# esw0116/DynaVSR

Hardware: AMD Instinct MI355X
Metric: inner-loop frames/sec/GPU (EDVR-M x4, 5x3x180x320): forward leg = BASELINE.json configs[1]; the inner MAML step and the per-frame pipeline are `inner_step` / `per_frame_pipeline` (higher is better)
Workload: dtype f32; 1 GPU; EDVR-M x4 forward (PCD deformable alignment + TSA fusion + reconstruction), clips of 1x5x3x180x320 -> 3x720x1280 (BASELINE.json configs[1]); one step = 2 clip(s) per GPU, one per HIP stream (adapt.super_resolve_video); clips_in_flight_per_gpu=2

## Files before the change

### dynavsr_amd/_lib.py

```python
import ctypes
import os
from ctypes import POINTER, Structure, c_char_p, c_float, c_int, c_longlong, c_size_t, c_void_p

import torch

_runtime = {"configured": False, "hw_queues": None, "effective": None}


def configure_runtime(hw_queues=6):
    if not _runtime["configured"]:
        user = os.environ.get("GPU_MAX_HW_QUEUES")
        late = torch.cuda.is_initialized()
        if user is None and not late:
            os.environ["GPU_MAX_HW_QUEUES"] = str(int(hw_queues))
        _runtime.update(configured=True, hw_queues=os.environ.get("GPU_MAX_HW_QUEUES"),
                        effective=(user is not None) or not late)
    return {"hw_queues": _runtime["hw_queues"], "effective": _runtime["effective"]}


def runtime_report(device=None):
    r = configure_runtime()
    overlaps = None
    if torch.cuda.is_available():
        with torch.cuda.device(device if device is not None else torch.cuda.current_device()):
            overlaps = int(lib().dvsr_side_stream_overlaps(stream()))
    return {"hw_queues": r["hw_queues"], "effective": r["effective"], "side_stream_overlaps": overlaps}


_HERE = os.path.dirname(os.path.abspath(__file__))
SO_PATH = os.path.join(_HERE, "libdynavsr_hip.so")
_lib = None

ACT_NONE, ACT_LRELU, ACT_RELU = 0, 1, 2


class Conv2dDesc(Structure):
    _fields_ = [("x0", c_void_p), ("x1", c_void_p), ("w", c_void_p), ("bias", c_void_p),
                ("res", c_void_p), ("y", c_void_p),
                ("N", c_int), ("c0", c_int), ("c1", c_int), ("H", c_int), ("W", c_int),
                ("Cout", c_int), ("ks", c_int), ("stride", c_int), ("pad", c_int), ("act", c_int),
                ("pixel_shuffle", c_int), ("x1_bdiv", c_int),
                ("x0_bstride", c_longlong), ("x1_bstride", c_longlong),
                ("pre", c_void_p), ("pre_bdiv", c_int)]


class EdvrConfig(Structure):
    _fields_ = [(k, c_int) for k in ("nf", "nframes", "groups", "front_RBs", "back_RBs", "scale",
                                     "center", "bf16_mfma")]


class FrameDesc(Structure):
    _fields_ = [("format", c_int), ("h", c_int), ("w", c_int), ("row_stride", c_longlong), ("plane_stride", c_longlong),
                ("pixel_stride", c_int)]


FRAME_F32_CHW, FRAME_U8_HWC_RGB, FRAME_U8_HWC_BGR, FRAME_U8_Y = 0, 1, 2, 3
FRAME_U16_Y_MSB, FRAME_U16_Y_10, FRAME_U16_Y_12 = 4, 5, 6
FRAME_PAD_REFLECT, FRAME_PAD_REPLICATE = 0, 1


class YuvDesc(Structure):
    _fields_ = [("format", c_int), ("h", c_int), ("w", c_int), ("matrix", c_int), ("range", c_int),
                ("plane", c_void_p * 3), ("row_stride", c_longlong * 3)]


YUV_NV12, YUV_I420 = 0, 1
YUV_CHROMA_420, YUV_CHROMA_422, YUV_CHROMA_444 = 0, 1, 2


def yuv_format(form, chroma):
    return form | (chroma << 4)


YUV_BT601, YUV_BT709 = 0, 1
YUV_LIMITED, YUV_FULL = 0, 1


class Yuv16Desc(Structure):
    _fields_ = [("format", c_int), ("depth", c_int), ("h", c_int), ("w", c_int), ("matrix", c_int), ("range", c_int),
                ("plane", c_void_p * 3), ("row_stride", c_longlong * 3)]


YUV16_SEMI_MSB, YUV16_PLANAR_LSB = 0, 1


class ResizeAxis(Structure):
    _fields_ = [("first", c_void_p), ("weights", c_void_p), ("taps", c_int)]


class StitchAxis(Structure):
    _fields_ = [("first", c_void_p), ("weights", c_void_p), ("origins", c_void_p), ("cover", c_int)]


FLIP_W, FLIP_H = 1, 2


class ScoreArgs(Structure):
    _fields_ = [("channel", c_int), ("crop_border", c_int), ("depth", c_int), ("lo", c_float), ("hi", c_float)]


SCORE_RGB, SCORE_Y = 0, 1


class EstimatorConfig(Structure):
    _fields_ = [(k, c_int) for k in ("kind", "nf", "in_nc", "scale", "nframes")]


def _declare(lib):
    P, I, F, LL = c_void_p, c_int, c_float, c_longlong
    sig = {
        "dvsr_last_error": (c_char_p, []),
        "dvsr_version": (I, []),
        "dvsr_mdcn_forward": (I, [P] * 6 + [I] * 13 + [P]),
        "dvsr_mdcn_forward_fast_workspace_bytes": (c_size_t, [I, I, I]),
        "dvsr_mdcn_forward_fast": (I, [P] * 6 + [I] * 7 + [P, c_size_t, P]),
        "dvsr_mdcn_pack_forward": (I, [P] * 5 + [I] * 13 + [P]),
        "dvsr_mdcn_pack_forward_fast": (I, [P] * 5 + [I] * 7 + [P, c_size_t, P]),
        "dvsr_conv2d_forward": (I, [POINTER(Conv2dDesc), P]),
        "dvsr_upsample_bilinear_forward": (I, [P, P, LL, I, I, I, F, P]),
        "dvsr_upsample_bilinear_backward": (I, [P, P, LL, I, I, I, F, I, P]),
        "dvsr_pool3s2_forward": (I, [P, P, P, LL, I, I, P]),
        "dvsr_pool3s2_backward": (I, [P, P, P, P, LL, I, I, P]),
        "dvsr_tsa_gate_forward": (I, [P] * 5 + [I, I, I, LL, P]),
        "dvsr_tsa_gate_backward": (I, [P] * 8 + [I, I, I, LL, P]),
        "dvsr_tsa_blend_forward": (I, [P] * 4 + [LL, P]),
        "dvsr_tsa_blend_backward": (I, [P] * 5 + [LL, P]),
        "dvsr_edvr_plan_create": (I, [POINTER(EdvrConfig), I, I, I, POINTER(c_void_p)]),
        "dvsr_edvr_plan_create_grouped": (I, [POINTER(EdvrConfig), I, I, I, I, POINTER(c_void_p)]),
        "dvsr_edvr_plan_create_ex": (I, [POINTER(EdvrConfig), I, I, I, I, I, POINTER(c_void_p)]),
        "dvsr_edvr_plan_destroy": (None, [P]),
        "dvsr_edvr_num_params": (I, [P]),
        "dvsr_edvr_num_launches": (I, [P]),
        "dvsr_edvr_workspace_bytes": (c_size_t, [P, I]),
        "dvsr_edvr_forward": (I, [P, POINTER(c_void_p), P, P, P, c_size_t, P]),
        "dvsr_edvr_forward_packed": (I, [P, POINTER(c_void_p), P, P, P, c_size_t, P]),
        "dvsr_edvr_backward": (I, [P, POINTER(c_void_p), P, P, POINTER(c_void_p), P, P, c_size_t, P]),
        "dvsr_edvr_num_backward_launches": (I, [P]),
        "dvsr_estimator_plan_create": (I, [POINTER(EstimatorConfig), I, I, I, POINTER(c_void_p)]),
        "dvsr_estimator_plan_create_grouped": (I, [POINTER(EstimatorConfig), I, I, I, I, POINTER(c_void_p)]),
        "dvsr_estimator_plan_create_ex": (I, [POINTER(EstimatorConfig), I, I, I, I, I, POINTER(c_void_p)]),
        "dvsr_estimator_plan_destroy": (None, [P]),
        "dvsr_estimator_num_params": (I, [P]),
        "dvsr_estimator_num_launches": (I, [P, I]),
        "dvsr_estimator_workspace_bytes": (c_size_t, [P, I]),
        "dvsr_estimator_forward": (I, [P, POINTER(c_void_p), P, P, P, c_size_t, P]),
        "dvsr_estimator_backward": (I, [P, POINTER(c_void_p), P, P, POINTER(c_void_p), P, c_size_t, P]),
        "dvsr_conv2d_backward_workspace_bytes": (c_size_t, [POINTER(Conv2dDesc)]),
        "dvsr_conv2d_backward": (I, [POINTER(Conv2dDesc), P, P, P, P, P, P, c_size_t, P]),
        "dvsr_mdcn_backward_workspace_bytes": (c_size_t, [I] * 10),
        "dvsr_mdcn_backward": (I, [P] * 10 + [I] * 12 + [P, c_size_t, P]),
        "dvsr_adam_step": (I, [POINTER(c_void_p)] * 4 + [POINTER(LL), I, F, F, F, F, F, I, P]),
        "dvsr_sgd_step": (I, [POINTER(c_void_p)] * 2 + [POINTER(LL), I, F, F, P]),
        "dvsr_replicate_tensors": (I, [POINTER(c_void_p)] * 2 + [POINTER(LL), I, I, P]),
        "dvsr_degrade_apply": (I, [P, P, P, I, I, I, I, I, I, I, I, I, P]),
        "dvsr_frame_metrics_workspace_bytes": (c_size_t, [I, I, I]),
        "dvsr_frame_metrics": (I, [P, P, I, I, I, F, F, P, P, P, c_size_t, P]),
        "dvsr_charbonnier_workspace_bytes": (c_size_t, []),
        "dvsr_charbonnier_forward": (I, [P, P, P, LL, F, P, c_size_t, P]),
        "dvsr_conv2d_packed_workspace_bytes": (c_size_t, [POINTER(Conv2dDesc)]),
        "dvsr_conv2d_forward_packed": (I, [POINTER(Conv2dDesc), P, c_size_t, P]),
        "dvsr_conv2d_dgrad_packed": (I, [POINTER(Conv2dDesc), P, P, P, c_size_t, P]),
        "dvsr_conv2d_packed_geometry": (I, [POINTER(Conv2dDesc), POINTER(ctypes.c_int * 4)]),
        "dvsr_conv2d_wgrad_geometry": (I, [POINTER(Conv2dDesc), I, I, POINTER(ctypes.c_int * 8)]),
        "dvsr_conv2d_wgrad_workspace_bytes": (c_size_t, [POINTER(Conv2dDesc), I]),
        "dvsr_conv2d_wgrad_bf16": (I, [POINTER(Conv2dDesc), P, P, P, P, c_size_t, P]),
        "dvsr_conv2d_wgrad_split3": (I, [POINTER(Conv2dDesc), P, P, P, P, c_size_t, P]),
        "dvsr_flow_warp_forward": (I, [P, P, P, I, I, I, I, LL, P]),
        "dvsr_flow_warp_backward": (I, [P, P, P, P, P, I, I, I, I, LL, P]),
        "dvsr_avgpool2_forward": (I, [P, P, LL, I, I, P]),
        "dvsr_avgpool2_backward": (I, [P, P, LL, I, I, I, P]),
        "dvsr_resize_bilinear_ac_forward": (I, [P, P, LL, I, I, I, I, F, LL, P]),
        "dvsr_resize_bilinear_ac_backward": (I, [P, P, LL, I, I, I, I, F, LL, P]),
        "dvsr_upsample_bicubic_ac_forward": (I, [P, P, LL, I, I, I, P]),
        "dvsr_upsample_bicubic_ac_backward": (I, [P, P, LL, I, I, I, P]),
        "dvsr_channel_affine": (I, [P, P, P, P, I, I, LL, LL, LL, I, P]),
        "dvsr_batchnorm_workspace_bytes": (c_size_t, [I]),
        "dvsr_batchnorm_forward": (I, [P] * 8 + [I, I, LL, I, F, F, I, P, c_size_t, P]),
        "dvsr_batchnorm_backward": (I, [P] * 9 + [I, I, LL, I, I, P, c_size_t, P]),
        "dvsr_temporal_gather3_forward": (I, [P, P, I, I, I, LL, I, P]),
        "dvsr_temporal_gather3_backward": (I, [P, P, I, I, I, LL, I, P]),
        "dvsr_dynamic_filter_forward": (I, [P, P, P, P, I, I, I, I, I, P]),
        "dvsr_dynamic_filter_backward": (I, [P, P, P, P, P, P, I, I, I, I, I, P]),
        "dvsr_conv3x3_small_cout": (I, [P, P, P, P, P, I, I, I, I, I, I, P]),
        "dvsr_conv1x1_dual": (I, [P, P, P, P, P, P, P, I, I, I, I, I, P]),
        "dvsr_patch_gather_forward": (I, [P, P, POINTER(c_int), POINTER(c_int), I, I, I, I, I, I, P]),
        "dvsr_patch_gather_backward": (I, [P, P, POINTER(c_int), POINTER(c_int), I, I, I, I, I, I, P]),
        "dvsr_l1_tail_forward": (I, [P, P, P, F, P, LL, P, c_size_t, P]),
        "dvsr_l1_tail_backward": (I, [P, P, P, F, P, LL, P]),
        "dvsr_charbonnier_backward": (I, [P, P, P, P, LL, F, P]),
        "dvsr_charbonnier_forward_grouped": (I, [P, P, P, LL, I, F, P, c_size_t, P]),
        "dvsr_charbonnier_backward_grouped": (I, [P, P, P, P, LL, I, F, P]),
        "dvsr_l1_tail_forward_grouped": (I, [P, P, P, F, P, LL, I, P, c_size_t, P]),
        "dvsr_l1_tail_backward_grouped": (I, [P, P, P, F, P, LL, I, P]),
        "dvsr_edvr_op_info": (I, [P, I, c_char_p, I, c_char_p, I, POINTER(ctypes.c_double),
                                  POINTER(ctypes.c_double)]),
        "dvsr_edvr_forward_timed": (I, [P, POINTER(c_void_p), P, P, P, c_size_t, P, POINTER(c_float)]),
        "dvsr_debug_mfma_peak": (LL, [P, I, I, I, I, P]),
        "dvsr_debug_mfma_shadow": (I, [P, P, I, I, I, I, I, P]),
        "dvsr_edvr_tensor_info": (I, [P, c_char_p, POINTER(LL), POINTER(LL)]),
        "dvsr_edvr_plan_work": (I, [P, POINTER(ctypes.c_double * 9)]),
        "dvsr_edvr_plan_work_nograd": (I, [P, POINTER(ctypes.c_double * 9)]),
        "dvsr_edvr_op_launch_count": (I, [P, I, I]),
        "dvsr_side_stream_overlaps": (I, [P]),
        "dvsr_edvr_op_output": (I, [P, I, I, POINTER(c_int), POINTER(LL), POINTER(LL)]),
        "dvsr_estimator_plan_work": (I, [P, POINTER(ctypes.c_double * 9)]),
        "dvsr_edvr_stream_create": (I, [POINTER(EdvrConfig), I, I, I, POINTER(c_void_p)]),
        "dvsr_edvr_stream_destroy": (None, [P]),
        "dvsr_edvr_stream_num_params": (I, [P]),
        "dvsr_edvr_stream_num_launches": (I, [P, I]),
        "dvsr_edvr_stream_cache_bytes": (c_size_t, [P]),
        "dvsr_edvr_stream_workspace_bytes": (c_size_t, [P]),
        "dvsr_edvr_stream_extract": (I, [P, POINTER(c_void_p), P, I, P, c_size_t, P, c_size_t, I, P]),
        "dvsr_edvr_stream_fuse": (I, [P, POINTER(c_void_p), POINTER(c_int), P, c_size_t, P, P, c_size_t, I, P]),
        "dvsr_frame_ingest": (I, [P, POINTER(FrameDesc), P, I, I, I, P]),
        "dvsr_frame_emit": (I, [P, I, I, P, POINTER(FrameDesc), F, F, P]),
        "dvsr_edvr_stream_extract_frame": (I, [P, POINTER(c_void_p), P, POINTER(FrameDesc), I, I, P, c_size_t, P, c_size_t, I,
                                               P]),
        "dvsr_frame_ingest_yuv": (I, [POINTER(YuvDesc), P, I, I, I, P]),
        "dvsr_frame_emit_yuv": (I, [P, I, I, POINTER(YuvDesc), F, F, P]),
        "dvsr_edvr_stream_extract_frame_yuv": (I, [P, POINTER(c_void_p), POINTER(YuvDesc), I, I, P, c_size_t, P, c_size_t, I, P]),
        "dvsr_frame_luma_sad": (I, [P, P, POINTER(FrameDesc), LL, I, P, P]),
        "dvsr_frame_ingest_yuv16": (I, [POINTER(Yuv16Desc), P, I, I, I, P]),
        "dvsr_frame_emit_yuv16": (I, [P, I, I, POINTER(Yuv16Desc), F, F, P]),
        "dvsr_edvr_stream_extract_frame_yuv16": (I, [P, POINTER(c_void_p), POINTER(Yuv16Desc), I, I, P, c_size_t, P, c_size_t, I,
                                                     P]),
        "dvsr_frame_resize_taps": (I, [I, I]),
        "dvsr_frame_resize_table": (I, [I, I, I, P, P]),
        "dvsr_frame_resize": (I, [P, I, I, I, I, P, I, I, I, I, POINTER(ResizeAxis), POINTER(ResizeAxis), P]),
        "dvsr_frame_flip": (I, [P, P, LL, I, I, I, P]),
        "dvsr_frame_flip_mean": (I, [P, P, P, P, P, LL, I, I, P]),
        "dvsr_frame_stitch_origins": (I, [I, I, I, POINTER(c_int), I]),
        "dvsr_frame_stitch_cover": (I, [I, I, I]),
        "dvsr_frame_stitch_table": (I, [I, I, I, I, I, P, P]),
        "dvsr_frame_stitch": (I, [P, I, I, I, I, I, P, I, I, POINTER(StitchAxis), POINTER(StitchAxis), POINTER(c_int),
                                  POINTER(c_int), P]),
        "dvsr_edvr_stream_max_image_bytes": (ctypes.c_ulonglong, [P]),
        "dvsr_frame_score_workspace_bytes": (c_size_t, [I, I, I]),
        "dvsr_frame_score": (I, [P, POINTER(FrameDesc), P, POINTER(FrameDesc), POINTER(ScoreArgs), P, P, c_size_t, P]),
    }
    for name, (res, args) in sig.items():
        fn = getattr(lib, name)
        fn.restype = res
        fn.argtypes = args
    return sig


def lib():
    global _lib
    if _lib is None:
        if not os.path.exists(SO_PATH):
            raise RuntimeError(
                "libdynavsr_hip.so is missing (%s). Build it with `python -m dynavsr_amd.build` "
                "(hipcc --offload-arch=gfx950); there is no fallback path." % SO_PATH)
        _lib = ctypes.CDLL(os.environ.get("DVSR_HIP_LIB", SO_PATH))
        _lib._signatures = _declare(_lib)
    return _lib


def check(rc, what=""):
    if rc != 0:
        msg = lib().dvsr_last_error().decode("utf-8", "replace")
        raise RuntimeError("libdynavsr_hip %s failed (rc=%d): %s" % (what, rc, msg))


def ptr(t):
    if t is None:
        return None
    if not t.is_cuda:
        raise RuntimeError("libdynavsr_hip needs a tensor on the GPU, got device %s" % t.device)
    if t.dtype != torch.float32:
        raise RuntimeError("libdynavsr_hip computes in fp32, got %s" % t.dtype)
    if not t.is_contiguous():
        raise RuntimeError("libdynavsr_hip needs contiguous tensors")
    return t.data_ptr()


def stream():
    return torch.cuda.current_stream().cuda_stream
```

### dynavsr_amd/csrc/conv2d_v2.hip

```cpp
#include <algorithm>
#include <cmath>
#include <cstdlib>
#include <type_traits>

#include "common.h"
#include "kernels.h"
#include "small_grid.h"

namespace dvsr {

#ifdef DVSR_CONV_TRACE
#define DVSR_ABLATE(a) ((a).ablate)
#define DVSR_STAMP(i)                                                                              \
  do {                                                                                             \
    if (a.trace && threadIdx.x == 0) a.trace[(size_t)blockIdx.x * 64 + (i)] = __builtin_readcyclecounter(); \
  } while (0)
#else
#define DVSR_ABLATE(a) 0
#define DVSR_STAMP(i) \
  do {                \
  } while (0)
#endif

template <int KS, int S, int CC, int TH, int MT, int BF = 0>
// ... 30 lines not shown
    const int hi = r & 1; r >>= 1;
    const int q = r % kq4; r /= kq4;
    const int tap = r % e.KK;
    const int mt = r / e.KK;
    const int co = cb * 64 + mt * 32 + lo, ci = k * e.CC + (e.layout != PackLayout::INTERLEAVED ? 8 * q + 4 * hi + j : 2 * (4 * q + j) + hi);
    float v = 0.f;
    if (co < e.Cout && ci < e.Ctot) {
      if (!e.wt) v = e.w[((size_t)co * e.Ctot + ci) * e.KK + tap];
      else v = e.w[((size_t)ci * e.w_ctot + e.w_coff + co) * e.KK + (e.KK - 1 - tap)];
    }
    e.P[i] = v;
  }
}

__global__ void pack_weights_bf16_kernel(PackTable t) {
  const PackEntry& e = t.e[blockIdx.y];
  if (!e.bf) return;
  const int kb = e.CC / 16;
  const size_t per_chunk = (size_t)e.pch * 2;
  const size_t total = (size_t)e.ncb * e.nchunks * per_chunk;
  __bf16* P16 = reinterpret_cast<__bf16*>(e.P);
  for (size_t i = blockIdx.x * (size_t)blockDim.x + threadIdx.x; i < total;
       i += (size_t)gridDim.x * blockDim.x) {
    int r = (int)(i % per_chunk);
    const size_t ck = i / per_chunk;
    const int k = (int)(ck % e.nchunks), cb = (int)(ck / e.nchunks);
    const int j = r & 7; r >>= 3;
    const int lo = r & 31; r >>= 5;
    const int hi = r & 1; r >>= 1;
    const int q = r % kb; r /= kb;
    const int tap = r % e.KK; r /= e.KK;
    const int mt = r & 1;
    const int piece = r >> 1;
    const int co = cb * 64 + mt * 32 + lo, ci = k * e.CC + 16 * q + 8 * hi + j;
    float v = 0.f;
    if (co < e.Cout && ci < e.Ctot) {
      if (!e.wt) v = e.w[((size_t)co * e.Ctot + ci) * e.KK + tap];
      else v = e.w[((size_t)ci * e.w_ctot + e.w_coff + co) * e.KK + (e.KK - 1 - tap)];
    }
    __bf16 out = (__bf16)v;
    if (piece > 0) {
      const float r1 = v - (float)out;
      const __bf16 m = (__bf16)r1;
      out = piece == 1 ? m : (__bf16)(r1 - (float)m);
    }
    P16[i] = out;
  }
}

int pack_weights_run(const PackTable& t, hipStream_t st) {
  auto any = [&](auto pred) {
    for (int i = 0; i < t.n; ++i) if (pred(t.e[i])) return true;
    return false;
  };
  for (int i = 0; i < t.n; ++i)
    DVSR_REQUIRE(t.e[i].wt || !t.e[i].w_ctot || (t.e[i].layout == PackLayout::WINO_F4 && !t.e[i].bf), DVSR_ERR_UNSUPPORTED,
                 "pack_weights: only the F(4x4) pack takes a slice of the input channels");
  const struct { PackLayout layout; int (*run)(const PackTable&, hipStream_t); } own[] = {
      {PackLayout::DCN_SPLIT, pack_weights_dcn3_run}, {PackLayout::WINO_F2, pack_weights_wino_run},
      {PackLayout::WINO_F2_BF16, pack_weights_wino3_run}, {PackLayout::WINO_F4, pack_weights_wino5_run}};
  for (const auto& o : own)
    if (any([&](const PackEntry& e) { return !e.bf && e.layout == o.layout; })) {
      int rc = o.run(t, st);
      if (rc) return rc;
    }
  if (any([](const PackEntry& e) { return !e.bf && !has_own_pack_kernel(e.layout); })) {
    hipLaunchKernelGGL(pack_weights_kernel, dim3(48, t.n), dim3(256), 0, st, t);
    int rc = check_launch("pack_weights_kernel");
    if (rc) return rc;
  }
  if (any([](const PackEntry& e) { return e.bf != 0; })) {
    hipLaunchKernelGGL(pack_weights_bf16_kernel, dim3(48, t.n), dim3(256), 0, st, t);
    return check_launch("pack_weights_bf16_kernel");
  }
  return DVSR_OK;
}

typedef __bf16 bf16x8 __attribute__((ext_vector_type(8)));

template <int KS, int S, int CC, int TH, int MT, int BF>
__device__ __forceinline__ void conv2d_pipe_item(const ConvK2& a, const int id, float* const smem) {
  using Sh = Conv2Shape<KS, S, CC, TH, MT, BF>;
  constexpr int KK = Sh::KK, IH = Sh::IH, IW = Sh::IW, PLANE = Sh::PLANE, E = Sh::E, KQ4 = Sh::KQ4,
                NT = Sh::NT;
  float* const s_in0 = smem;
  float* const s_w0 = smem + Sh::IN_FLOATS;

  const int q_ = id >> 3;
  const int cbi = q_ % a.ncb;
  const int j_ = q_ / a.ncb;
  const int tile = (id & 7) * a.tiles_per_xcd + j_;
  if (j_ >= a.tiles_per_xcd || tile >= a.ntiles) return;
  const int tx_ = tile % a.tiles_x;
  const int t2 = tile / a.tiles_x;
  const int ty_ = t2 % a.tiles_y;
  const int n = t2 / a.tiles_y;
  const int oy0 = ty_ * TH, ox0 = tx_ * Sh::TW;
  const int iy0 = oy0 * S - a.pad, ix0 = ox0 * S - a.pad;

  const int tid = threadIdx.x, lane = tid & 63;
  const int wave = __builtin_amdgcn_readfirstlane(tid >> 6);
  const int lo = lane & 31, hi = lane >> 5;
  const int Ctot = a.c0 + a.c1;
  const size_t HW = (size_t)a.H * a.W;
  const float* x0n = a.x0 + (size_t)n * a.x0_bs;
  const float* x1n = a.c1 ? a.x1 + (size_t)(n / a.x1_bdiv) * a.x1_bs : x0n;
  const size_t cstride0 = a.in_dil ? (size_t)a.Hs * a.Ws : HW;

  unsigned eoffb[E];
  int elds[E];
  bool evalid[E];
#pragma unroll
  for (int e = 0; e < E; ++e) {
    const int idx = tid + 256 * e;
    const int iy = idx / IW, ix = idx - iy * IW;
    elds[e] = (iy * 2) * IW + ix;
    const int gy = iy0 + iy, gx = ix0 + ix;
    bool ok = idx < PLANE && (unsigned)gy < (unsigned)a.H && (unsigned)gx < (unsigned)a.W;
    int off = gy * a.W + gx;
    if (a.in_ps) off = (2 * gy) * (2 * a.W) + 2 * gx;
    if (a.in_dil) {
      ok = ok && !((gy | gx) & 1) && (gy >> 1) < a.Hs && (gx >> 1) < a.Ws;
      off = (gy >> 1) * a.Ws + (gx >> 1);
    }
    eoffb[e] = ok ? (unsigned)off * 4u : 0u;
    evalid[e] = ok;
  }

  f32x16 acc[MT][NT];
#pragma unroll
  for (int i = 0; i < MT; ++i)
#pragma unroll
    for (int j = 0; j < NT; ++j)
#pragma unroll
      for (int r = 0; r < 16; ++r) acc[i][j][r] = 0.f;

  float rin[CC][E];
  constexpr int PIECES = Sh::PIECES;
  const float* wp_cb = wset_ptr(a.wp, a.w_gs, n, a.wdiv) + ((size_t)((cbi * MT) >> 1) * a.nchunks * PIECES * 2 + ((cbi * MT) & 1)) * Sh::HALF;

  auto issue_halo = [&](int k) {
    const int cbase = k * CC;
    const bool second = cbase >= a.c0;
    const float* b = second ? x1n : x0n;
    const int ci = second ? cbase - a.c0 : cbase;
    const size_t cs = second ? HW : cstride0;
    const char* p = reinterpret_cast<const char*>(b + (size_t)ci * cs);
    const size_t inc0 = a.in_ps ? 4 : cs * 4;
    const size_t inc1 = a.in_ps ? ((size_t)2 * a.W - 1) * 4 : cs * 4;
    const size_t inc3 = a.in_ps ? ((size_t)4 * HW - 2 * a.W - 1) * 4 : cs * 4;
#pragma unroll
    for (int c = 0; c < CC; ++c) {
#pragma unroll
      for (int e = 0; e < E; ++e) rin[c][e] = *reinterpret_cast<const float*>(p + eoffb[e]);
      if (c + 1 < CC) {
        const size_t inc = (c & 1) == 0 ? inc0 : ((c & 3) == 1 ? inc1 : inc3);
        p += (cbase + c + 1 < Ctot) ? inc : 0;
      }
    }
  };
  auto issue_dma = [&](int k, int buf) {
    if constexpr (Sh::AG) return;
    const float* wsrc = wp_cb + (size_t)k * (PIECES * 2 * Sh::HALF);
    float* wdst = s_w0 + buf * Sh::BUF_FLOATS;
    constexpr int NP1 = Sh::W1 / 256;
#pragma unroll
    for (int j = 0; j < (Sh::NPIECE + 3) / 4; ++j) {
      int piece = j * 4 + wave;
      piece = piece < Sh::NPIECE ? piece : Sh::NPIECE - 1;
      const int op = piece / (NP1 > 0 ? NP1 : 1), within = piece - op * NP1;
      __builtin_amdgcn_global_load_lds(
          (const __attribute__((address_space(1))) void*)(wsrc + op * (2 * Sh::HALF) + within * 256 + lane * 4),
          (__attribute__((address_space(3))) void*)(wdst + op * Sh::W1 + within * 256), 16, 0, 0);
    }
  };
  auto write_halo = [&](int k, int buf) {
    float* s_in = s_in0 + buf * Sh::BUF_FLOATS;
#pragma unroll
    for (int e = 0; e < E; ++e) {
      if (tid + 256 * e < PLANE) {
#pragma unroll
        for (int q = 0; q < KQ4; ++q)
#pragma unroll
          for (int h2 = 0; h2 < 2; ++h2) {
            const bool ev = evalid[e];
            f32x4 v;
            if (BF == 2) {
              const int cb0 = k * CC + 16 * q + 8 * h2;
              bf16x8 p0, p1, p2;
#pragma unroll
              for (int i = 0; i < 8; ++i) {
                const float x = (ev && cb0 + i < Ctot) ? rin[16 * q + 8 * h2 + i][e] : 0.f;
                const __bf16 h = (__bf16)x;
                const float r1 = x - (float)h;
                const __bf16 m = (__bf16)r1;
                p0[i] = h; p1[i] = m; p2[i] = (__bf16)(r1 - (float)m);
              }
              float* dst = s_in + ((size_t)(q * IH * 2 * IW) + elds[e] + h2 * IW) * 4;
              *reinterpret_cast<f32x4*>(dst + Sh::IN1) = __builtin_bit_cast(f32x4, p1);
              *reinterpret_cast<f32x4*>(dst + 2 * Sh::IN1) = __builtin_bit_cast(f32x4, p2);
              v = __builtin_bit_cast(f32x4, p0);
            } else if (BF) {
              const int cb0 = k * CC + 16 * q + 8 * h2;
              bf16x8 hv;
#pragma unroll
              for (int i = 0; i < 8; ++i) hv[i] = (__bf16)((ev && cb0 + i < Ctot) ? rin[16 * q + 8 * h2 + i][e] : 0.f);
              v = __builtin_bit_cast(f32x4, hv);
            } else {
              const int cb0 = k * CC + 8 * q + h2;
              v = f32x4{(ev && cb0 < Ctot) ? rin[8 * q + h2][e] : 0.f,
                        (ev && cb0 + 2 < Ctot) ? rin[8 * q + 2 + h2][e] : 0.f,
                        (ev && cb0 + 4 < Ctot) ? rin[8 * q + 4 + h2][e] : 0.f,
                        (ev && cb0 + 6 < Ctot) ? rin[8 * q + 6 + h2][e] : 0.f};
            }
            *reinterpret_cast<f32x4*>(s_in + ((size_t)(q * IH * 2 * IW) + elds[e] + h2 * IW) * 4) = v;
          }
      }
    }
  };

  constexpr int NSTEP = KK * KQ4;
  constexpr int SPLIT = (3 * NSTEP) / 4;
  constexpr int RING = NSTEP % 3 == 0 ? 3 : 2;
  static_assert(!Sh::AG || (NSTEP % RING == 0 && KQ4 == 1), "the register ring of the global-A path needs NSTEP % RING == 0");
  constexpr int AD = 1;
  f32x4 Ag[Sh::AG ? RING : 1][MT][PIECES];
  auto load_a = [&](int k, int tap, int slot) {
    const float* b = wp_cb + (size_t)k * (PIECES * 2 * Sh::HALF) + tap * 256 + lane * 4;
#pragma unroll
    for (int op = 0; op < PIECES; ++op)
#pragma unroll
      for (int mt = 0; mt < MT; ++mt)
        Ag[slot][mt][op] = *reinterpret_cast<const f32x4*>(b + (op * 2 + mt) * Sh::HALF);
  };
  auto block = [&](int k, auto has_next_tag) {
    constexpr bool HAS_NEXT = decltype(has_next_tag)::value;
    const int buf = k & 1;
    const float* s_in = s_in0 + buf * Sh::BUF_FLOATS;
    const float* s_w = s_w0 + buf * Sh::BUF_FLOATS;
    if (k < 8) DVSR_STAMP(2 + 4 * k);
    if (HAS_NEXT && !Sh::AG) {
      issue_dma(k + 1, buf ^ 1);
      issue_halo(k + 1);
      __builtin_amdgcn_sched_barrier(0);
    }
    if (k < 8) DVSR_STAMP(3 + 4 * k);
    f32x4 A[2][Sh::AG ? 1 : MT][PIECES], Bv[Sh::AG ? 1 : 2][NT][PIECES];
    auto load_ops = [&](int step, int rb) {
      const int tap = step / KQ4, q = step - tap * KQ4;
      const int ty = tap / KS, tx = tap - ty * KS;
#pragma unroll
      for (int op = 0; op < PIECES; ++op) {
        if constexpr (!Sh::AG) {
#pragma unroll
          for (int mt = 0; mt < MT; ++mt)
            A[rb][mt][op] = *reinterpret_cast<const f32x4*>(
                s_w + op * Sh::W1 + ((size_t)((((mt * KK + tap) * KQ4 + q) * 2 + hi) * 32 + lo)) * 4);
        }
#pragma unroll
        for (int nt = 0; nt < NT; ++nt)
          Bv[rb][nt][op] = *reinterpret_cast<const f32x4*>(
              s_in + op * Sh::IN1 + ((size_t)(((q * IH + (NT * wave + nt) * S + ty) * 2 + hi) * IW + lo * S + tx)) * 4);
      }
    };
    auto load_b = [&](int step, int op) {
      const int ty = step / KS, tx = step - ty * KS;
#pragma unroll
      for (int nt = 0; nt < NT; ++nt)
        Bv[0][nt][op] = *reinterpret_cast<const f32x4*>(
            s_in + op * Sh::IN1 + ((size_t)((((NT * wave + nt) * S + ty) * 2 + hi) * IW + lo * S + tx)) * 4);
    };
    if constexpr (Sh::AG) { load_b(0, 2); load_b(0, 1); load_b(0, 0); }
    else load_ops(0, 0);
#pragma unroll
    for (int step = 0; step < NSTEP; ++step) {
      const int rb = step & 1;
      if constexpr (Sh::AG) {
        if (step + AD < NSTEP) load_a(k, step + AD, (step + AD) % RING);
        else if (HAS_NEXT) load_a(k + 1, step + AD - NSTEP, (step + AD) % RING);
        if (HAS_NEXT && step == 0) issue_halo(k + 1);
        __builtin_amdgcn_sched_barrier(0);
      }
      if (!Sh::AG && step + 1 < NSTEP) load_ops(step + 1, rb ^ 1);
      if (HAS_NEXT && step == SPLIT) {
        if (k < 8) DVSR_STAMP(4 + 4 * k);
        __builtin_amdgcn_sched_barrier(0);
        write_halo(k + 1, buf ^ 1);
        __builtin_amdgcn_sched_barrier(0);
        if (k < 8) DVSR_STAMP(5 + 4 * k);
      }
      if constexpr (BF == 2) {
        auto mm = [&](int pa, int pb) {
#pragma unroll
          for (int mt = 0; mt < MT; ++mt)
#pragma unroll
            for (int nt = 0; nt < NT; ++nt)
              acc[mt][nt] = __builtin_amdgcn_mfma_f32_32x32x16_bf16(
                  __builtin_bit_cast(bf16x8, Ag[step % RING][mt][pa]), __builtin_bit_cast(bf16x8, Bv[0][nt][pb]),
                  acc[mt][nt], 0, 0, 0);
        };
        mm(0, 2);
        if (step + 1 < NSTEP) { load_b(step + 1, 2); __builtin_amdgcn_sched_barrier(0); }
        mm(1, 1);
        mm(0, 1);
        if (step + 1 < NSTEP) { load_b(step + 1, 1); __builtin_amdgcn_sched_barrier(0); }
        mm(2, 0);
        mm(1, 0);
        mm(0, 0);
        if (step + 1 < NSTEP) { load_b(step + 1, 0); __builtin_amdgcn_sched_barrier(0); }
      } else if (BF) {
#pragma unroll
        for (int mt = 0; mt < MT; ++mt)
#pragma unroll
          for (int nt = 0; nt < NT; ++nt)
            acc[mt][nt] = __builtin_amdgcn_mfma_f32_32x32x16_bf16(__builtin_bit_cast(bf16x8, A[rb][mt][0]),
                                                                  __builtin_bit_cast(bf16x8, Bv[rb][nt][0]), acc[mt][nt],
                                                                  0, 0, 0);
      } else {
#pragma unroll
        for (int j = 0; j < 4; ++j)
#pragma unroll
          for (int mt = 0; mt < MT; ++mt)
#pragma unroll
            for (int nt = 0; nt < NT; ++nt)
              acc[mt][nt] = __builtin_amdgcn_mfma_f32_32x32x2f32(A[rb][mt][0][j], Bv[rb][nt][0][j], acc[mt][nt], 0, 0, 0);
      }
    }
    if (HAS_NEXT) __syncthreads();
  };

  DVSR_STAMP(0);
#ifdef DVSR_CONV_TRACE
  if (a.trace && threadIdx.x == 0) a.trace[(size_t)blockIdx.x * 64 + 60] = __builtin_amdgcn_s_memrealtime();
#endif
  issue_dma(0, 0);
  if constexpr (Sh::AG) {
#pragma unroll
    for (int i = 0; i < AD; ++i) load_a(0, i, i);
  }
  issue_halo(0);
  write_halo(0, 0);
  DVSR_STAMP(1);
  __syncthreads();
  for (int k = 0; k + 1 < a.nchunks; ++k) block(k, std::true_type{});
  block(a.nchunks - 1, std::false_type{});

  DVSR_STAMP(40);
  const TileOut t{a.y, wset_ptr(a.bias, a.b_gs, n, a.wdiv), a.res, a.act, a.ps, a.accum, a.Cout, a.Ho, a.Wo, a.gmask, a.gmask_act};
  store_mfma_tile<MT, NT>(acc, t, n, cbi * MT * 32, oy0, TH, ox0, oy0 + NT * wave, lo, hi);
#ifdef DVSR_CONV_TRACE
  DVSR_STAMP(41);
  __builtin_amdgcn_s_waitcnt(0);
  DVSR_STAMP(42);
  if (a.trace && threadIdx.x == 0) a.trace[(size_t)blockIdx.x * 64 + 61] = __builtin_amdgcn_s_memrealtime();
  if (a.trace && threadIdx.x == 0)
    a.trace[(size_t)blockIdx.x * 64 + 63] = __builtin_amdgcn_s_getreg((4) | (0 << 6) | (31 << 11));
#endif
}

template <int KS, int S, int CC, int TH, int MT, int BF = 0>
__global__ __launch_bounds__(256, (BF == 2 && TH == 4) ? 3 : 2) void conv2d_pipe_kernel(ConvK2 a) {
  extern __shared__ __attribute__((aligned(16))) float smem[];
  conv2d_pipe_item<KS, S, CC, TH, MT, BF>(a, blockIdx.x, smem);
}

template <int KS, int S, int CC, int TH, int MT, int BF = 0>
static int launch_conv2(ConvK2 k, hipStream_t st) {
  using Sh = Conv2Shape<KS, S, CC, TH, MT, BF>;
  auto kern = conv2d_pipe_kernel<KS, S, CC, TH, MT, BF>;
  static PerDeviceOnce attr_once;
  size_t lds = Sh::LDS_BYTES;
#ifdef DVSR_CONV_TRACE
  if (const char* e = getenv("DVSR_CONV_LDS")) lds = std::max(lds, (size_t)atol(e));
#endif
  set_dyn_lds_once(attr_once, (const void*)kern, lds);
  k.tiles_x = ceil_div(k.Wo, 32); k.tiles_y = ceil_div(k.Ho, TH); k.ntiles = k.tiles_x * k.tiles_y * k.N;
  k.ncb = ceil_div(k.Cout, 32 * MT);
  k.tiles_per_xcd = ceil_div(k.ntiles, 8);
  k.nitems = k.tiles_per_xcd * 8 * k.ncb;
  const int grid = k.nitems;
  hipLaunchKernelGGL(kern, dim3(grid), dim3(256), lds, st, k);
  return check_launch("conv2d_pipe_kernel");
}


template <int TH, int MT>
struct DmaShape {
  static constexpr int KK = 9, CC = 8, NT = TH / 4, IH = TH + 2, RP = 40, GR = RP / 4;
  static constexpr int NG = CC * IH * GR;
  static constexpr int NI = (NG + 255) / 256;
  static constexpr int IN_FLOATS = NG * 4;
  static constexpr int HALF = KK * 2 * 32 * 4;
  static constexpr int W_FLOATS = MT * HALF;
  static constexpr int NPIECE = W_FLOATS / 256;
  static constexpr int BUF_FLOATS = IN_FLOATS + W_FLOATS;
  static constexpr size_t LDS_BYTES = (size_t)2 * BUF_FLOATS * sizeof(float);
};

template <int TH, int MT>
__device__ __forceinline__ void conv2d_dma_item(const ConvK2& a, const int id, float* const smem) {
  using Sh = DmaShape<TH, MT>;
  constexpr int KK = Sh::KK, CC = Sh::CC, IH = Sh::IH, NT = Sh::NT, RP = Sh::RP, GR = Sh::GR, NI = Sh::NI;
  float* const s_in0 = smem;
  float* const s_w0 = smem + Sh::IN_FLOATS;

  const int q_ = id >> 3;
  const int cbi = q_ % a.ncb;
  const int j_ = q_ / a.ncb;
  const int tile = (id & 7) * a.tiles_per_xcd + j_;
  if (j_ >= a.tiles_per_xcd || tile >= a.ntiles) return;
  const int tx_ = tile % a.tiles_x;
  const int t2 = tile / a.tiles_x;
  const int ty_ = t2 % a.tiles_y;
  const int n = t2 / a.tiles_y;
  const int oy0 = ty_ * TH, ox0 = tx_ * 32;

  const int tid = threadIdx.x, lane = tid & 63;
  const int wave = __builtin_amdgcn_readfirstlane(tid >> 6);
  const int lo = lane & 31, hi = lane >> 5;
  const size_t HW = (size_t)a.H * a.W;
  const float* x0n = a.x0 + (size_t)n * a.x0_bs;
  const float* x1n = a.c1 ? a.x1 + (size_t)(n / a.x1_bdiv) * a.x1_bs : x0n;

  unsigned hoff[NI];
  bool hval[NI];
#pragma unroll
  for (int jj = 0; jj < NI; ++jj) {
    const int L = 64 * (wave + 4 * jj) + lane;
    const int c = L / (IH * GR), r = L - c * (IH * GR);
    const int iy = r / GR, g = r - iy * GR;
    const int gy = oy0 - 1 + iy, gx = ox0 - 4 + 4 * g;
    const bool ok = L < Sh::NG && (unsigned)gy < (unsigned)a.H && (unsigned)gx < (unsigned)a.W;
    hoff[jj] = ok ? (unsigned)(((size_t)c * HW + (size_t)gy * a.W + gx) * 4) : 0u;
    hval[jj] = ok;
    if (L < Sh::NG && !ok) {
      *reinterpret_cast<f32x4*>(s_in0 + L * 4) = f32x4{0.f, 0.f, 0.f, 0.f};
      *reinterpret_cast<f32x4*>(s_in0 + Sh::BUF_FLOATS + L * 4) = f32x4{0.f, 0.f, 0.f, 0.f};
    }
  }

  f32x16 acc[MT][NT];
#pragma unroll
  for (int i = 0; i < MT; ++i)
#pragma unroll
    for (int j = 0; j < NT; ++j)
#pragma unroll
      for (int r = 0; r < 16; ++r) acc[i][j][r] = 0.f;

  const float* wp_cb = wset_ptr(a.wp, a.w_gs, n, a.wdiv) + ((size_t)((cbi * MT) >> 1) * a.nchunks * 2 + ((cbi * MT) & 1)) * Sh::HALF;

  auto issue_halo = [&](int k, int buf) {
    const int cbase = k * CC;
    const bool second = cbase >= a.c0;
    const float* b = second ? x1n : x0n;
    const int ci = second ? cbase - a.c0 : cbase;
    const char* p = reinterpret_cast<const char*>(b + (size_t)ci * HW);
    float* dst = s_in0 + buf * Sh::BUF_FLOATS;
#pragma unroll
    for (int jj = 0; jj < NI; ++jj) {
      if (hval[jj])
        __builtin_amdgcn_global_load_lds((const __attribute__((address_space(1))) void*)(p + hoff[jj]),
                                         (__attribute__((address_space(3))) void*)(dst + 256 * (wave + 4 * jj)), 16, 0, 0);
    }
  };
  auto issue_w = [&](int k, int buf) {
    const float* wsrc = wp_cb + (size_t)k * (2 * Sh::HALF);
    float* wdst = s_w0 + buf * Sh::BUF_FLOATS;
#pragma unroll
    for (int j = 0; j < (Sh::NPIECE + 3) / 4; ++j) {
      int piece = j * 4 + wave;
      piece = piece < Sh::NPIECE ? piece : Sh::NPIECE - 1;
      __builtin_amdgcn_global_load_lds((const __attribute__((address_space(1))) void*)(wsrc + piece * 256 + lane * 4),
                                       (__attribute__((address_space(3))) void*)(wdst + piece * 256), 16, 0, 0);
    }
  };

  const int bbase = (4 * hi * IH + NT * wave) * RP + lo + 3;
  auto block = [&](int k, auto has_next_tag) {
    constexpr bool HAS_NEXT = decltype(has_next_tag)::value;
    const int buf = k & 1;
    const float* s_in = s_in0 + buf * Sh::BUF_FLOATS + bbase;
    const float* s_w = s_w0 + buf * Sh::BUF_FLOATS;
    if (HAS_NEXT) {
      if (!(DVSR_ABLATE(a) & 4)) issue_w(k + 1, buf ^ 1);
      if (!(DVSR_ABLATE(a) & 2)) issue_halo(k + 1, buf ^ 1);
      __builtin_amdgcn_sched_barrier(0);
    }
    f32x4 A[2][MT];
    float Bv[2][NT][4];
    auto load_ops = [&](int tap, int rb) {
      const int ty = tap / 3, tx = tap - ty * 3;
#pragma unroll
      for (int mt = 0; mt < MT; ++mt)
        A[rb][mt] = *reinterpret_cast<const f32x4*>(s_w + ((size_t)(((mt * KK + tap) * 2 + hi) * 32 + lo)) * 4);
#pragma unroll
      for (int nt = 0; nt < NT; ++nt)
#pragma unroll
        for (int j = 0; j < 4; ++j) Bv[rb][nt][j] = s_in[(j * IH + nt + ty) * RP + tx];
    };
    load_ops(0, 0);
// ... 167 lines not shown
    float Bv[2][NT][4];
    auto load_ops = [&](int kx, int rb) {
#pragma unroll
      for (int mt = 0; mt < MT; ++mt)
        A[rb][mt] = *reinterpret_cast<const f32x4*>(s_w + ((size_t)(((mt * KS + kx) * 2 + hi) * 32 + lo)) * 4);
#pragma unroll
      for (int nt = 0; nt < NT; ++nt)
#pragma unroll
        for (int j = 0; j < 4; ++j) Bv[rb][nt][j] = s_in[(j * IH + nt) * RP + kx];
    };
    load_ops(0, 0);
#pragma unroll
    for (int kx = 0; kx < KS; ++kx) {
      const int rb = kx & 1;
      if (kx + 1 < KS) load_ops(kx + 1, rb ^ 1);
#pragma unroll
      for (int j = 0; j < 4; ++j)
#pragma unroll
        for (int mt = 0; mt < MT; ++mt)
#pragma unroll
          for (int nt = 0; nt < NT; ++nt)
            acc[mt][nt] = __builtin_amdgcn_mfma_f32_32x32x2f32(A[rb][mt][j], Bv[rb][nt][j], acc[mt][nt], 0, 0, 0);
    }
    if (has_next) __syncthreads();
    if (++ky == KS) { ky = 0; ++k; }
  }

  const TileOut t{a.y, wset_ptr(a.bias, a.b_gs, n, a.wdiv), a.res, a.act, a.ps, a.accum, a.Cout, a.Ho, a.Wo, a.gmask, a.gmask_act};
  store_mfma_tile<MT, NT>(acc, t, n, cbi * MT * 32, oy0, TH, ox0, oy0 + NT * wave, lo, hi);
}

template <int KS, int TH, int MT>
static int launch_dmarow(ConvK2 k, hipStream_t st) {
  using Sh = RowShape<KS, TH, MT>;
  auto kern = conv2d_dmarow_kernel<KS, TH, MT>;
  static PerDeviceOnce attr_once;
  set_dyn_lds_once(attr_once, (const void*)kern, Sh::LDS_BYTES);
  k.tiles_x = ceil_div(k.Wo, 32); k.tiles_y = ceil_div(k.Ho, TH); k.ntiles = k.tiles_x * k.tiles_y * k.N;
  k.ncb = ceil_div(k.Cout, 32 * MT);
  k.tiles_per_xcd = ceil_div(k.ntiles, 8);
  k.nitems = k.tiles_per_xcd * 8 * k.ncb;
  hipLaunchKernelGGL(kern, dim3(k.nitems), dim3(256), Sh::LDS_BYTES, st, k);
  return check_launch("conv2d_dmarow_kernel");
}

template <int MT, int NT>
__global__ __launch_bounds__(256, 2) void conv2d_ksplit_kernel(ConvK2 a) {
  extern __shared__ __attribute__((aligned(16))) float smem[];
  conv2d_ksplit_item<MT, NT>(a, blockIdx.x, smem);
}

template <int MT, int NT>
static int launch_ksplit(ConvK2 k, hipStream_t st) {
  using Sh = KsShape<MT, NT>;
  auto kern = conv2d_ksplit_kernel<MT, NT>;
  static PerDeviceOnce attr_once;
  set_dyn_lds_once(attr_once, (const void*)kern, Sh::LDS_BYTES);
  hipLaunchKernelGGL(kern, dim3(k.nitems), dim3(256), Sh::LDS_BYTES, st, k);
  return check_launch("conv2d_ksplit_kernel");
}

namespace {
struct ConvShape { int ks, stride, N, Ho, Wo, Cout, Ctot; };
int int_or(const char* v, int dflt) { return v ? atoi(v) : dflt; }

double conv2_pipe_cost(int TH, int MT, int CC, const ConvShape& s) {
  const double wgs = (double)ceil_div(s.Wo, 32) * ceil_div(s.Ho, TH) * s.N * ceil_div(s.Cout, 32 * MT);
  return ceil(wgs / 256.0) * 64.0 * (s.ks * s.ks) * (CC / 2) * (TH / 4) * MT;
}
bool mt1_wins(int cc, const ConvShape& s) { return conv2_pipe_cost(4, 1, cc, s) < 0.97 * conv2_pipe_cost(4, 2, cc, s); }

ConvGeo choose_row_split(const ConvShape& s, ConvAllow allow) {
  ConvGeo g{8, 4, mt1_wins(8, s) ? 1 : 2};
  if ((allow & ALLOW_DMA_HALO) && s.stride == 1 && s.Wo % 4 == 0) g.kernel = ConvKernel::ROW_SPLIT;
  return g;
}

constexpr long long KSPLIT_BELOW_WGS = 700;
bool choose_ksplit(const ConvShape& s, ConvAllow allow, ConvGeo* g) {
  if (!(s.ks == 3 && s.stride == 1 && (allow & ALLOW_KSPLIT) && s.Ctot >= 32 && s.Cout >= 32)) return false;
  const long long wg41 = (long long)ceil_div(s.Wo, 32) * ceil_div(s.Ho, 4) * s.N * ceil_div(s.Cout, 32);
  if (wg41 >= KSPLIT_BELOW_WGS) return false;
  *g = (s.Cout % 64 != 0 && s.Ho % 2 == 0) ? ConvGeo{32, 2, 1} : ConvGeo{32, 1, 2};
  return true;
}

int chunk_channels(int ks) { return ks == 1 ? 32 : (ks == 2 ? 16 : 8); }
ConvGeo choose_direct_tile(const ConvShape& s) {
  const int cc = chunk_channels(s.ks);
  if (s.ks == 3 && s.stride == 2) {
    const double c82 = conv2_pipe_cost(8, 2, cc, s);
    if (c82 <= conv2_pipe_cost(4, 2, cc, s) && c82 <= conv2_pipe_cost(4, 1, cc, s)) return ConvGeo{cc, 8, 2};
  }
  return ConvGeo{cc, 4, mt1_wins(cc, s) ? 1 : 2};
}

struct WinoPick { int th; double cost; };
double wino_workgroups(const ConvShape& s, int oh, int ow) { return (double)ceil_div(s.Wo, ow) * ceil_div(s.Ho, oh) * s.N * ceil_div(s.Cout, 64); }
double wino_rounds_cost(const ConvShape& s, double cus, int oh, int ow, double chunk_cyc, double fixed_cyc) {
  return ceil(wino_workgroups(s, oh, ow) / cus) * ((s.Ctot / 8) * chunk_cyc + fixed_cyc) / 2.07;
}
double direct_cost(const ConvShape& s) {
  const double dcyc = std::min(conv2_pipe_cost(4, 2, 8, s), conv2_pipe_cost(4, 1, 8, s));
  const double drounds = dcyc / (64.0 * 9 * 4 * (mt1_wins(8, s) ? 1 : 2));
  return dcyc * (s.Ctot / 8) / (drounds <= 6.0 ? 0.60 : 0.78) / 2.4;
}
WinoPick wino_f2_cost(const ConvShape& s, double cus, bool tile16) {
  const double w4 = wino_rounds_cost(s, cus, 4, 64, 5100.0, 12500.0), w8 = wino_rounds_cost(s, cus, 8, 32, 5100.0, 12500.0);
  const double w16 = tile16 ? wino_rounds_cost(s, cus, 16, 16, 5100.0, 12500.0) : 1e300;
  return {(w16 < w4 && w16 < w8) ? 16 : (w8 < w4 ? 8 : 4), std::min(std::min(w4, w8), w16)};
}
constexpr double W5_CHUNK_CYC = 4300.0, W5_FIXED_CYC = 17500.0;
WinoPick wino_f4_cost(const ConvShape& s, double cus) {
  const double f8 = wino_rounds_cost(s, cus, 8, 64, W5_CHUNK_CYC, W5_FIXED_CYC), f16 = wino_rounds_cost(s, cus, 16, 32, W5_CHUNK_CYC, W5_FIXED_CYC);
  return {f16 < f8 ? 16 : 8, std::min(f8, f16)};
}
constexpr double SHARED_LATENCY_BOUND = 1.05;
bool f4_occupies_less(const ConvShape& s, double cus, const WinoPick& f2, const WinoPick& f4) {
  const int ow2 = f2.th == 16 ? 16 : (f2.th == 8 ? 32 : 64), ow4 = f4.th == 16 ? 32 : 64;
  const double g2 = wino_workgroups(s, f2.th, ow2), g4 = wino_workgroups(s, f4.th, ow4);
  if (g2 > cus || g4 > cus) return false;
  ConvShape one = s;
  one.N = 1;
  if (2.0 * wino_workgroups(one, f2.th, ow2) <= cus || 2.0 * wino_workgroups(one, f4.th, ow4) > cus) return false;
  return g4 * f4.cost < g2 * f2.cost && f4.cost <= SHARED_LATENCY_BOUND * f2.cost;
}
}

double conv2_f4_occupied_cycles(int N, int Ho, int Wo, int Cout, int Ctot, int th) {
  const ConvShape s{3, 1, N, Ho, Wo, Cout, Ctot};
  return wino_workgroups(s, th, th == 16 ? 32 : 64) * ((Ctot / 8) * W5_CHUNK_CYC + W5_FIXED_CYC);
}

ConvGeo conv2_choose(int ks, int stride, int N, int Ho, int Wo, int Cout, int Ctot, ConvAllow allow) {
  const ConvShape s{ks, stride, N, Ho, Wo, Cout, Ctot};
  if (ks == 7 || ks == 9) return choose_row_split(s, allow);
  ConvGeo g;
  if (choose_ksplit(s, allow, &g)) return g;
  g = choose_direct_tile(s);
  if ((allow & ALLOW_DMA_HALO) && ks == 3 && stride == 1 && Wo % 4 == 0 && Ctot % 8 == 0) g.kernel = ConvKernel::DMA_HALO;
  const int wino_on = int_or(getenv("DVSR_CONV_WINO"), 1);
  if (!(wino_on && g.kernel == ConvKernel::DMA_HALO && (allow & ALLOW_WINO) && Cout >= 32 && Ctot >= 16)) return g;
  const int wino3_on = int_or(getenv("DVSR_CONV_WINO3"), 1), wino5_on = int_or(getenv("DVSR_CONV_WINO5"), 1);
  const double direct = direct_cost(s), cus = (double)device_cus();
  const WinoPick f2 = wino_f2_cost(s, cus, wino3_on != 0);
  if (wino5_on && wino3_on && (allow & ALLOW_WINO_F4) && Wo % 4 == 0 && device_lds_optin() >= (size_t)156 * 1024) {
    const WinoPick f4 = wino_f4_cost(s, cus);
    const bool shared_pick = (allow & ALLOW_SHARED_DEVICE) && f2.cost < direct && f4_occupies_less(s, cus, f2, f4);
    if (wino5_on >= 2 || (allow & ALLOW_ONLY_F4) || ((1.15 * f4.cost < f2.cost || shared_pick) && f4.cost < direct))
      return ConvGeo{8, wino5_on == 3 ? 16 : f4.th, 2, 0, ConvKernel::WINO_F4};
  }
  if ((wino_on == 2 || f2.cost < direct) && device_lds_optin() >= (size_t)155 * 1024)
    return ConvGeo{8, f2.th, 2, 0, wino3_on ? ConvKernel::WINO_F2_BF16 : ConvKernel::WINO_F2};
  return g;
}

static int pack_chunk_floats(int ks, int cc, int bf, PackLayout layout) {
  switch (layout) {
    case PackLayout::WINO_F2: return 16 * 2 * 64 * 4;
    case PackLayout::WINO_F2_BF16: return 2 * 6144;
    case PackLayout::WINO_F4: return 18 * 2 * 3 * 256;
    case PackLayout::DCN_SPLIT: return mdcn_pack_floats();
    default: return (bf == 2 ? 3 : 1) * 2 * ks * ks * (bf ? cc / 16 : cc / 8) * 2 * 32 * 4;
  }
}
size_t conv2_pack_floats(int ks, int Cout, int Ctot, int cc, int bf, PackLayout layout) {
  return (size_t)ceil_div(Cout, 64) * ceil_div(Ctot, cc) * pack_chunk_floats(ks, cc, bf, layout);
}
PackEntry conv2_pack_entry(const float* w, float* P, int ks, int Cout, int Ctot, int cc, int bf, PackLayout layout, int wt, int w_ctot,
                           int w_coff) {
  PackEntry e{};
  e.w = w; e.P = P; e.Cout = Cout; e.Ctot = Ctot; e.KK = ks * ks; e.CC = cc; e.wt = wt; e.w_ctot = w_ctot; e.w_coff = w_coff;
  e.ncb = ceil_div(Cout, 64); e.nchunks = ceil_div(Ctot, cc); e.pch = pack_chunk_floats(ks, cc, bf, layout);
  e.bf = bf; e.layout = layout;
  return e;
}

#ifdef DVSR_CONV_TRACE
static long long* g_trace_buf = nullptr;
static int g_trace_countdown = -1;
extern "C" int dvsr_debug_conv_trace(void* buf, int launch_index) {
  g_trace_buf = (long long*)buf;
  g_trace_countdown = launch_index;
  return 0;
}
#endif

int conv2d_packed_prepare(const dvsr_conv2d_desc& d, const float* wp, const ConvExtra& ex, const ConvGeo& geo, ConvK2* out) {
  DVSR_REQUIRE(d.x0 && wp && d.y, DVSR_ERR_INVALID, "conv2d_packed: null x0/wp/y");
  DVSR_REQUIRE(((d.ks == 1 || d.ks == 2) && d.stride == 1) || (d.ks == 3 && (d.stride == 1 || d.stride == 2)) ||
                   ((d.ks == 7 || d.ks == 9) && d.stride == 1 && geo.kernel == ConvKernel::ROW_SPLIT),
               DVSR_ERR_UNSUPPORTED, "conv2d_packed: ks=%d stride=%d", d.ks, d.stride);
  DVSR_REQUIRE(d.c1 == 0 || (d.c0 % geo.cc == 0 && !ex.in_ps && !ex.in_dil), DVSR_ERR_UNSUPPORTED,
               "conv2d_packed: two inputs need c0 %% %d == 0 and a plain first input (c0=%d)", geo.cc, d.c0);
  ConvK2& k = *out;
  k.x0 = d.x0; k.x1 = d.x1; k.wp = wp; k.bias = d.bias; k.res = d.res; k.y = d.y;
  k.N = d.N; k.c0 = d.c0; k.c1 = d.c1; k.H = d.H; k.W = d.W; k.Cout = d.Cout;
  k.pad = d.pad; k.act = d.act; k.ps = d.pixel_shuffle; k.x1_bdiv = d.x1_bdiv > 0 ? d.x1_bdiv : 1;
  k.x0_bs = d.x0_bstride > 0 ? d.x0_bstride : (long long)d.c0 * d.H * d.W;
  k.x1_bs = d.x1_bstride > 0 ? d.x1_bstride : (long long)d.c1 * d.H * d.W;
  k.Ho = (d.H + 2 * d.pad - d.ks) / d.stride + 1;
  k.Wo = (d.W + 2 * d.pad - d.ks) / d.stride + 1;
  k.nchunks = ceil_div(d.c0 + d.c1, geo.cc);
  k.in_ps = ex.in_ps; k.in_dil = ex.in_dil; k.Hs = ex.Hs; k.Ws = ex.Ws; k.accum = ex.accum;
  k.gmask = ex.gmask; k.gmask_act = ex.gmask_act;
  k.wdiv = ex.wdiv > 0 ? ex.wdiv : 1; k.w_gs = ex.w_gs; k.b_gs = ex.b_gs;
  DVSR_REQUIRE(!d.pre || (geo.kernel == ConvKernel::WINO_F4 && !d.res && d.pixel_shuffle == 0 && ((uintptr_t)d.pre & 15) == 0),
               DVSR_ERR_UNSUPPORTED, "conv2d_packed: a pre-activation addend needs the F(4x4, 3x3) kernel, a 16-byte aligned tensor, "
               "no residual and no PixelShuffle");
  k.pre = d.pre; k.pre_bdiv = d.pre_bdiv > 0 ? d.pre_bdiv : 1; k.pre_bs = (long long)d.Cout * k.Ho * k.Wo;
#ifdef DVSR_CONV_TRACE
  {
    static int ablate = -1;
    if (ablate < 0) {
      const char* v = getenv("DVSR_CONV_ABLATE");
      ablate = v ? atoi(v) : 0;
    }
    k.ablate = ablate;
  }
#endif
  if (k.in_ps) k.x0_bs = (long long)d.c0 * d.H * d.W;
  if (k.in_dil) k.x0_bs = (long long)d.c0 * ex.Hs * ex.Ws;
#ifdef DVSR_CONV_TRACE
  k.trace = (g_trace_countdown == 0) ? g_trace_buf : nullptr;
  if (g_trace_countdown >= 0) --g_trace_countdown;
#endif
  if (geo.kernel == ConvKernel::ROW_SPLIT) {
    DVSR_REQUIRE((d.ks == 7 || d.ks == 9) && d.stride == 1 && d.pad == d.ks / 2 && !ex.in_ps && !ex.in_dil && geo.cc == 8 &&
                     geo.th == 4 && d.W % 4 == 0 && (d.c1 == 0 || d.c0 % 8 == 0) && k.x0_bs % 4 == 0 && k.x1_bs % 4 == 0 &&
                     ((uintptr_t)d.x0 & 15) == 0 && ((uintptr_t)d.x1 & 15) == 0,
                 DVSR_ERR_UNSUPPORTED, "conv2d_packed: the row-split DMA kernel needs 7x7 / 9x9, stride 1, pad ks/2, plain "
                 "16-byte aligned inputs and W %% 4 == 0 (W=%d c0=%d c1=%d)", d.W, d.c0, d.c1);
  } else if (needs_dma_halo_inputs(geo.kernel)) {
    DVSR_REQUIRE(!is_winograd(geo.kernel) || d.c0 + d.c1 >= 16, DVSR_ERR_UNSUPPORTED, "conv2d_packed: the Winograd kernel needs two 8-channel chunks");
    DVSR_REQUIRE(geo.kernel != ConvKernel::WINO_F4 || (!ex.accum && !ex.gmask && d.W % 4 == 0 && (geo.th == 8 || geo.th == 16)), DVSR_ERR_UNSUPPORTED,
                 "conv2d_packed: the F(4x4, 3x3) kernel stores whole tile columns of forward launches (W=%d th=%d)", d.W, geo.th);
    DVSR_REQUIRE(!is_winograd(geo.kernel) || d.pixel_shuffle == 0 || (d.pixel_shuffle == 2 && d.Cout % 4 == 0 && !d.res && !ex.accum && !ex.gmask),
                 DVSR_ERR_UNSUPPORTED, "conv2d_packed: the Winograd kernel stores plain or PixelShuffle(2) tiles (ps=%d)", d.pixel_shuffle);
    DVSR_REQUIRE(d.ks == 3 && d.stride == 1 && d.pad == 1 && !ex.in_ps && !ex.in_dil && geo.cc == 8 && (geo.th == 4 || geo.th == 8 || (geo.th == 16 && on_bf16_split(geo.kernel))) &&
                     d.W % 4 == 0 && d.c0 % 8 == 0 && d.c1 % 8 == 0 && k.x0_bs % 4 == 0 && k.x1_bs % 4 == 0 &&
                     ((uintptr_t)d.x0 & 15) == 0 && ((uintptr_t)d.x1 & 15) == 0,
                 DVSR_ERR_UNSUPPORTED, "conv2d_packed: the DMA-halo kernel needs 3x3/s1/pad 1, plain 16-byte aligned inputs, "
                 "W %% 4 == 0 and channel counts %% 8 == 0 (W=%d c0=%d c1=%d)", d.W, d.c0, d.c1);
  }
  if (d.ks == 3 && geo.cc == 32) {
    DVSR_REQUIRE(d.stride == 1 && (d.c1 == 0 || d.c0 % 32 == 0) && !ex.in_ps && !ex.in_dil && d.pad == 1 &&
                     ((geo.th == 1 && geo.mt == 2) || (geo.th == 2 && geo.mt == 1)),
                 DVSR_ERR_UNSUPPORTED, "conv2d_packed: the K-split kernel needs 3x3/s1/pad 1, plain inputs, c0 %% 32 == 0 "
                 "with two inputs (th=%d mt=%d)", geo.th, geo.mt);
    k.tiles_x = ceil_div(k.Wo, 32); k.tiles_y = ceil_div(k.Ho, geo.th); k.ntiles = k.tiles_x * k.tiles_y * k.N;
    k.ncb = ceil_div(k.Cout, 32 * geo.mt);
    k.tiles_per_xcd = ceil_div(k.ntiles, 8);
    k.nitems = k.tiles_per_xcd * 8 * k.ncb;
  }
  return DVSR_OK;
}

template <int KS, int S, int CC, int TH, int BF>
static int launch_conv2_mt(int mt, const ConvK2& k, hipStream_t st) {
  return mt == 2 ? launch_conv2<KS, S, CC, TH, 2, BF>(k, st) : launch_conv2<KS, S, CC, TH, 1, BF>(k, st);
}

int conv2d_packed_run(const dvsr_conv2d_desc& d, const float* wp, const ConvExtra& ex, const ConvGeo& geo,
                      hipStream_t st) {
  ConvK2 k;
  int rc = conv2d_packed_prepare(d, wp, ex, geo, &k);
  if (rc) return rc;
  if (geo.bf) {
    DVSR_REQUIRE((d.ks == 3 || (d.ks == 2 && geo.bf == 2)) && d.stride == 1 && geo.cc == 16 && (geo.th == 4 || (geo.bf == 2 && geo.th == 8)),
                 DVSR_ERR_UNSUPPORTED,
                 "conv2d_packed: the bf16 kernel exists for 3x3 (split: also 2x2) stride-1 convs with 16-channel chunks");
    const bool th8 = geo.th == 8;
    if (geo.bf == 2 && d.ks == 2)
      return th8 ? launch_conv2_mt<2, 1, 16, 8, 2>(geo.mt, k, st) : launch_conv2_mt<2, 1, 16, 4, 2>(geo.mt, k, st);
    if (geo.bf == 2) return th8 ? launch_conv2_mt<3, 1, 16, 8, 2>(geo.mt, k, st) : launch_conv2_mt<3, 1, 16, 4, 2>(geo.mt, k, st);
    return launch_conv2_mt<3, 1, 16, 4, 1>(geo.mt, k, st);
  }
  switch (geo.kernel) {
    case ConvKernel::WINO_F2: return conv2d_wino_launch(k, geo.th, st);
    case ConvKernel::WINO_F2_BF16: return conv2d_wino3_launch(k, geo.th, st);
    case ConvKernel::WINO_F4: return conv2d_wino5_launch(k, geo.th, st);
    case ConvKernel::ROW_SPLIT:
      if (d.ks == 7) return geo.mt == 2 ? launch_dmarow<7, 4, 2>(k, st) : launch_dmarow<7, 4, 1>(k, st);
      return geo.mt == 2 ? launch_dmarow<9, 4, 2>(k, st) : launch_dmarow<9, 4, 1>(k, st);
    case ConvKernel::DMA_HALO:
      if (geo.th != 4) break;
      return geo.mt == 2 ? launch_dma<4, 2>(k, st) : launch_dma<4, 1>(k, st);
    case ConvKernel::REG:
      if (d.ks == 3 && geo.cc == 32) return geo.mt == 2 ? launch_ksplit<2, 1>(k, st) : launch_ksplit<1, 2>(k, st);
      switch (((d.ks * 10 + d.stride) * 100 + geo.cc) * 100 + geo.th * 10 + geo.mt) {
        case 320882: return launch_conv2<3, 2, 8, 8, 2>(k, st);
        case 320842: return launch_conv2<3, 2, 8, 4, 2>(k, st);
        case 320841: return launch_conv2<3, 2, 8, 4, 1>(k, st);
        case 310842: return launch_conv2<3, 1, 8, 4, 2>(k, st);
        case 310841: return launch_conv2<3, 1, 8, 4, 1>(k, st);
        case 211642: return launch_conv2<2, 1, 16, 4, 2>(k, st);
        case 211641: return launch_conv2<2, 1, 16, 4, 1>(k, st);
        case 113242: return launch_conv2<1, 1, 32, 4, 2>(k, st);
        case 113241: return launch_conv2<1, 1, 32, 4, 1>(k, st);
      }
      break;
  }
  DVSR_REQUIRE(false, DVSR_ERR_INVALID, "conv2d_packed: no kernel for ks=%d cc=%d th=%d mt=%d", d.ks, geo.cc, geo.th,
               geo.mt);
}

}

namespace {
struct OpPack {
  dvsr::ConvGeo geo;
  size_t floats;
};
OpPack op_pack(int ks, int stride, int pad, int N, int Ho, int Wo, int Cout, int Ctot, bool plain, bool aligned = false,
               bool only_f4 = false) {
  using namespace dvsr;
  OpPack o;
  const bool k3 = ks == 3 && stride == 1 && pad == 1, kbig = (ks == 7 || ks == 9) && stride == 1 && pad == ks / 2;
  o.geo = conv2_choose(ks, stride, N, Ho, Wo, Cout, Ctot, (k3 && plain && !only_f4 ? ALLOW_KSPLIT : ALLOW_NONE) | ((k3 || kbig) && aligned ? ALLOW_DMA_HALO : ALLOW_NONE) |
                                                              (k3 && aligned ? ALLOW_WINO | ALLOW_WINO_F4 : ALLOW_NONE) | (only_f4 ? ALLOW_ONLY_F4 : ALLOW_NONE));
  o.floats = conv2_pack_floats(ks, Cout, Ctot, o.geo);
  return o;
}
OpPack op_pack_for(const dvsr_conv2d_desc& d, int Cout, int Ctot) {
  const bool big = d.ks == 7 || d.ks == 9;
  const bool aligned = (((uintptr_t)d.x0 | (uintptr_t)d.x1) & 15) == 0 && (big ? (d.c1 == 0 || d.c0 % 8 == 0) : (d.c0 % 8 == 0 && d.c1 % 8 == 0)) &&
                       d.x0_bstride % 4 == 0 && d.x1_bstride % 4 == 0 && (d.H * d.W) % 4 == 0;
  return op_pack(d.ks, 1, d.pad, d.N, d.H, d.W, Cout, Ctot, d.c1 == 0 || d.c0 % 32 == 0, aligned, d.pre != nullptr);
}
int op_run(const dvsr_conv2d_desc& d, const dvsr::ConvExtra& ex, int Cout, int Ctot, void* ws, size_t bytes, hipStream_t st) {
  using namespace dvsr;
  DVSR_REQUIRE((d.ks == 1 || d.ks == 3 || d.ks == 7 || d.ks == 9) && d.stride == 1 && d.pad == d.ks / 2, DVSR_ERR_UNSUPPORTED,
               "conv2d (packed): ks=%d stride=%d pad=%d (1x1 / 3x3 / 7x7 / 9x9, stride 1, pad ks/2)", d.ks, d.stride, d.pad);
  const OpPack o = op_pack_for(d, Cout, Ctot);
  DVSR_REQUIRE(d.ks <= 3 || o.geo.kernel == ConvKernel::ROW_SPLIT, DVSR_ERR_UNSUPPORTED, "conv2d (packed): this %dx%d convolution is not eligible for the "
               "row-split kernel (dvsr_conv2d_packed_geometry): use dvsr_conv2d_forward / _backward", d.ks, d.ks);
  DVSR_REQUIRE(!d.pre || (o.geo.kernel == ConvKernel::WINO_F4 && !d.res && !d.pixel_shuffle), DVSR_ERR_UNSUPPORTED,
               "conv2d (packed): a pre-activation addend (pre) needs a launch the F(4x4, 3x3) kernel takes -- an aligned 3x3 / "
               "stride 1 / pad 1 convolution, W %% 4 == 0, whole 8-channel chunks, at least 32 outputs and 16 inputs -- without a "
               "residual or a PixelShuffle");
  DVSR_REQUIRE(ws && bytes >= o.floats * sizeof(float), DVSR_ERR_WORKSPACE, "conv2d (packed): workspace %zu < %zu bytes", bytes,
               o.floats * sizeof(float));
  PackTable t;
  t.n = 1;
  t.e[0] = conv2_pack_entry(d.w, (float*)ws, d.ks, Cout, Ctot, o.geo, ex.wt, ex.w_ctot, ex.w_coff);
  int rc = pack_weights_run(t, st);
  if (rc) return rc;
  return conv2d_packed_run(d, (const float*)ws, ex, o.geo, st);
}
}

extern "C" size_t dvsr_conv2d_packed_workspace_bytes(const dvsr_conv2d_desc* d) {
  if (!d || (d->ks != 1 && d->ks != 3 && d->ks != 7 && d->ks != 9)) return 0;
  const int ctot = d->c0 + d->c1;
  const size_t a = op_pack(d->ks, 1, d->ks / 2, d->N, d->H, d->W, d->Cout, ctot, true).floats;
  const size_t b = op_pack(d->ks, 1, d->ks / 2, d->N, d->H, d->W, ctot, d->Cout, true).floats;
  const size_t c = op_pack(d->ks, 1, d->ks / 2, d->N, d->H, d->W, d->Cout, ctot, false).floats;
  size_t w = 0;
  if (d->ks == 3)
    for (const dvsr::PackLayout l : {dvsr::PackLayout::WINO_F2_BF16, dvsr::PackLayout::WINO_F4})
      w = std::max(w, std::max(dvsr::conv2_pack_floats(3, d->Cout, ctot, 8, 0, l), dvsr::conv2_pack_floats(3, ctot, d->Cout, 8, 0, l)));
  return std::max(std::max(a, b), std::max(c, w)) * sizeof(float);
}

extern "C" int dvsr_conv2d_packed_geometry(const dvsr_conv2d_desc* d, int geo[4]) {
  DVSR_REQUIRE(d && geo && (d->ks == 1 || d->ks == 3 || d->ks == 7 || d->ks == 9) && d->stride == 1 && d->pad == d->ks / 2,
               DVSR_ERR_INVALID, "conv2d_packed_geometry: 1x1 / 3x3 / 7x7 / 9x9 stride-1 descriptors only");
  const OpPack o = op_pack_for(*d, d->Cout, d->c0 + d->c1);
  geo[0] = o.geo.cc; geo[1] = o.geo.th; geo[2] = o.geo.mt; geo[3] = static_cast<int>(o.geo.kernel);
  return DVSR_OK;
}

extern "C" int dvsr_conv2d_forward_packed(const dvsr_conv2d_desc* d, void* workspace, size_t workspace_bytes,
                                          dvsr_stream_t stream) {
  DVSR_REQUIRE(d && d->x0 && d->w && d->y, DVSR_ERR_INVALID, "conv2d_forward_packed: null argument");
  DVSR_REQUIRE(d->pixel_shuffle == 0 || (d->pixel_shuffle == 2 && d->Cout % 4 == 0 && !d->res), DVSR_ERR_INVALID,
               "conv2d_forward_packed: pixel_shuffle needs Cout %% 4 == 0 and no residual");
  return op_run(*d, dvsr::ConvExtra(), d->Cout, d->c0 + d->c1, workspace, workspace_bytes, (hipStream_t)stream);
}

extern "C" int dvsr_conv2d_dgrad_packed(const dvsr_conv2d_desc* d, const float* gy, float* gx0, void* workspace,
                                        size_t workspace_bytes, dvsr_stream_t stream) {
  using namespace dvsr;
  DVSR_REQUIRE(d && gy && gx0 && d->w, DVSR_ERR_INVALID, "conv2d_dgrad_packed: null argument");
  DVSR_REQUIRE(d->c1 == 0 && d->pixel_shuffle == 0, DVSR_ERR_UNSUPPORTED, "conv2d_dgrad_packed: single plain input only");
  dvsr_conv2d_desc g = {};
  g.x0 = gy; g.w = d->w; g.y = gx0; g.N = d->N; g.c0 = d->Cout; g.Cout = d->c0; g.H = d->H; g.W = d->W; g.ks = d->ks;
  g.stride = 1; g.pad = d->ks / 2; g.act = ACT_NONE; g.x1_bdiv = 1;
  ConvExtra ex;
  ex.wt = 1; ex.w_ctot = d->c0; ex.w_coff = 0;
  return op_run(g, ex, d->c0, d->Cout, workspace, workspace_bytes, (hipStream_t)stream);
}
```

### dynavsr_amd/csrc/engine.hip

```cpp
#include <algorithm>
#include <cstdlib>
#include <string>
#include <vector>

#include "common.h"
#include "kernels.h"
#include "small_grid.h"

namespace dvsr {

enum { SP_ARENA = 0, SP_INPUT = 1, SP_OUTPUT = 2, SP_NONE = 3 };
struct T {
  int space = SP_NONE;
  size_t off = 0, numel = 0;
  bool valid() const { return space != SP_NONE; }
};

enum OpType { OP_CONV, OP_DCN, OP_UP, OP_POOL, OP_GATE, OP_BLEND, OP_ADD, OP_PAD, OP_MEANSUB, OP_ADDMEAN };

struct Op {
  OpType type;
  const char* name = "";
  T x0, x1, res, y, y2;
  int pw = -1, pb = -1;
// ... 1 lines not shown
  int x1_bdiv = 1, dg = 8;
  int pad = -1;
  int pmode = 0, T = 1;
  int wmap = 0;
  size_t w2_off = 0;
  int no_dgrad = 0;
  int pad_out = 0;
  struct T ypad;
  int fused_into = -1;
  int dual = -1;
  long long x0_bs = 0, x1_bs = 0;
  int S = 1;
  float mul = 1.f;
  size_t planes = 0;
  int gB = 0, gN = 0, gC = 0;
  size_t gHW = 0;
  struct PackSlot { ConvGeo geo = {8, 8, 2}; size_t off = 0, floats = 0; };
  PackSlot dgrad[2], dcn_pack;
  enum LaunchRole { WHOLE, MAIN_PART, REF_PART };
  struct Launch { PackSlot pack; int c_off = 0, c = 0; LaunchRole role = WHOLE; };
  struct LaunchList {
    int n = 0; Launch l[2];
    const Launch* begin() const { return l; }
    const Launch* end() const { return l + n; }
    const Launch& primary() const { return l[n - 1]; }
  } launches[2];
  struct T pre;
};
enum FwdMode { FWD_GRAD = 0, FWD_NOGRAD = 1 };

enum { R_ACT = 0, R_GRAD = 1, R_X = 2, R_GX = 3, R_GOUT = 4, R_TMP = 5, R_NONE = 6 };
struct Ref {
  int space = R_NONE;
  size_t off = 0;
};
enum BType { B_MEMSET, B_COPYADD, B_ACT, B_WGRAD, B_DGRAD, B_REDUCE, B_DCN, B_UP, B_POOL, B_GATE, B_BLEND,
             B_PADFOLD, B_ADDMEAN, B_WUNMAP };
struct BOp {
  BType type;
  int fwd = -1;
  Ref a, b, c, d, e, f;
  size_t n = 0;
  int accum = 0, which = 0, cnt = 1, B = 0;
  int mask_op = -1;
  size_t ws_off = 0, ws_bytes = 0;
  long long bs = 0;
  size_t per = 0;
};

static inline int conv_pad(const Op& o) { return o.pad < 0 ? o.ks / 2 : o.pad; }
static inline int conv_out(const Op& o, int in) { return (in + 2 * conv_pad(o) - o.ks) / o.stride + 1; }

}

struct dvsr_edvr_plan {
  dvsr_edvr_config cfg;
  int B, H, W;
  int n_params = 0;
  size_t arena_floats = 0;
  std::vector<dvsr::Op> ops;
  std::vector<std::pair<std::string, dvsr::T>> named;
  std::vector<std::pair<size_t, size_t>> allocs;
  std::vector<dvsr::BOp> bops;
  size_t dpack_floats = 0;
  bool use_v1 = false;
  size_t tmp_floats = 0;
  size_t scratch_bytes = 0;
  size_t wscratch_bytes = 0;
  mutable hipStream_t side = nullptr;
  mutable hipEvent_t ev_fork = nullptr, ev_join = nullptr;
  int side_streams = 1;
  int fork_every = 3;
  const char* bwd_unsupported = nullptr;
  int wgroups = 1;
  int wsets = 1;
  bool split_any_pad = false;
};

namespace dvsr {

static T arena_alloc(dvsr_edvr_plan& p, const char* name, size_t numel) {
  T t;
  t.space = SP_ARENA;
  t.off = p.arena_floats;
  t.numel = numel;
  p.allocs.emplace_back(t.off, numel);
  p.arena_floats += (numel + 63) & ~(size_t)63;
  if (name && *name) p.named.emplace_back(name, t);
  return t;
}

static WgradDesc wgrad_shape(const dvsr_edvr_plan& p, const Op& o, int which) {
  WgradDesc d;
  d.x_bs = which ? o.x1_bs : o.x0_bs; d.x_bdiv = which ? o.x1_bdiv : 1; d.gy_ps = o.ps;
  d.N = o.N; d.Cin = which ? o.c1 : o.c0; d.H = o.H; d.W = o.W; d.Cout = o.Cout;
  d.Ctot = o.c0 + o.c1; d.c_off = which ? o.c0 : 0;
  d.ks = o.ks; d.stride = o.stride; d.pad = conv_pad(o);
  d.groups = p.wgroups; d.dW_gs = (long long)o.Cout * (o.c0 + o.c1) * o.ks * o.ks; d.db_gs = o.Cout;
  d.mode = (p.cfg.bf16_mfma == 1 && !o.wmap) ? 1 : (wgrad_split3_default() ? 2 : 0);
  return d;
}

static Op::LaunchList plan_hoist(const Op& o, const dvsr_edvr_plan& p, ConvAllow fwd_ok, const Op::Launch& whole) {
  Op::LaunchList pair;
  const char* hv = getenv("DVSR_PCD_HOIST");
  if ((hv && hv[0] == '0') || p.use_v1 || p.wsets != 1 || whole.pack.geo.kernel != ConvKernel::WINO_F4 || o.x1_bdiv <= 1 || o.c1 <= 0 ||
      o.N % o.x1_bdiv != 0 || o.res.valid() || o.ps)
    return pair;
  const int Ho = conv_out(o, o.H), Wo = conv_out(o, o.W), bd = o.x1_bdiv;
  const ConvAllow shared = fwd_ok | ALLOW_WINO_F4 | ALLOW_SHARED_DEVICE;
  const ConvAllow only_f4 = without(fwd_ok, ALLOW_KSPLIT) | ALLOW_WINO_F4 | ALLOW_ONLY_F4;
  auto choose = [&](int n, int c, ConvAllow allow) { return conv2_choose(o.ks, o.stride, n, Ho, Wo, o.Cout, c, allow); };
  auto f4 = [](const ConvGeo& g) { return g.kernel == ConvKernel::WINO_F4; };
  const ConvGeo gm = choose(o.N, o.c0, shared), gr = choose(o.N / bd, o.c1, only_f4);
  const ConvGeo u1 = choose(bd, o.c0 + o.c1, shared), m1 = choose(bd, o.c0, shared), r1 = choose(1, o.c1, only_f4);
  if (f4(gm) && f4(gr) && f4(u1) && f4(m1) && f4(r1) &&
      conv2_f4_occupied_cycles(bd, Ho, Wo, o.Cout, o.c0, m1.th) + conv2_f4_occupied_cycles(1, Ho, Wo, o.Cout, o.c1, r1.th) <
          conv2_f4_occupied_cycles(bd, Ho, Wo, o.Cout, o.c0 + o.c1, u1.th)) {
    const size_t mf = conv2_pack_floats(o.ks, o.Cout, o.c0, gm), rf = conv2_pack_floats(o.ks, o.Cout, o.c1, gr);
    if (mf + rf <= whole.pack.floats)
      pair = {2, {{{gr, whole.pack.off + mf, rf}, o.c0, o.c1, Op::REF_PART}, {{gm, whole.pack.off, mf}, 0, o.c0, Op::MAIN_PART}}};
  }
  return pair;
}

static void plan_conv_launches(Op& o, dvsr_edvr_plan& p) {
  const int ks = o.ks, N = o.N, c0 = o.c0, c1 = o.c1, Cout = o.Cout, Ho = conv_out(o, o.H), Wo = conv_out(o, o.W);
  const char* s2 = getenv("DVSR_EST_SPLIT2");
  const int split2 = s2 ? atoi(s2) : 1;
  const bool bf = p.cfg.bf16_mfma && (ks == 3 || (ks == 2 && p.split_any_pad && p.cfg.bf16_mfma == 2 && split2 && c0 % 16 == 0)) &&
                  o.stride == 1 && (o.pad < 0 || p.split_any_pad) && (c1 == 0 || c0 % 16 == 0);
  static const int split_th8_from = getenv("DVSR_SPLIT_TH8_FROM") ? atoi(getenv("DVSR_SPLIT_TH8_FROM")) : 200;
  auto as_bf = [&](ConvGeo g, int ho, int wo, int cout, bool dgrad = false) {
    if (!bf || (ks == 2 && split2 == 2 && dgrad)) return g;
    if (ks == 2 && (long long)ceil_div(wo, 32) * ceil_div(ho, 4) * N * ceil_div(cout, 64) < 256) return g;
    g.cc = 16; g.th = 4; g.bf = p.cfg.bf16_mfma == 2 ? 2 : 1;
    if (g.bf == 2 && (long long)ceil_div(wo, 32) * ceil_div(ho, 8) * N * ceil_div(cout, 32 * g.mt) >= split_th8_from)
      g.th = 8;
    return g;
  };
  const bool plain = o.pad < 0 && !o.wmap && !p.cfg.bf16_mfma;
  const ConvAllow ks_ok = (plain && (c1 == 0 || c0 % 32 == 0) ? ALLOW_KSPLIT : ALLOW_NONE) |
                          (plain && c0 % 8 == 0 && c1 % 8 == 0 ? ALLOW_DMA_HALO | ALLOW_WINO : ALLOW_NONE);
  const ConvAllow fwd_ok = (o.ps == 0 || (o.ps == 2 && !o.res.valid())) ? ks_ok : without(ks_ok, ALLOW_WINO);
  auto whole = [&](const ConvGeo& g) {
    const size_t floats = conv2_pack_floats(ks, Cout, c0 + c1, g);
    return Op::Launch{{g, arena_alloc(p, "", floats * p.wsets).off, floats}, 0, c0 + c1, Op::WHOLE};
  };
  o.launches[FWD_GRAD] = {1, {whole(as_bf(conv2_choose(ks, o.stride, N, Ho, Wo, Cout, c0 + c1, fwd_ok), Ho, Wo, Cout))}};
  Op::LaunchList& nograd = o.launches[FWD_NOGRAD] = o.launches[FWD_GRAD];
  if ((fwd_ok & ALLOW_WINO) && !nograd.l[0].pack.geo.bf) {
    const ConvGeo g5 = conv2_choose(ks, o.stride, N, Ho, Wo, Cout, c0 + c1, fwd_ok | ALLOW_WINO_F4 | ALLOW_SHARED_DEVICE);
    if (g5.kernel == ConvKernel::WINO_F4) nograd.l[0] = whole(g5);
  }
  const Op::LaunchList pair = plan_hoist(o, p, fwd_ok, nograd.l[0]);
  if (pair.n) {
    o.pre = arena_alloc(p, "", (size_t)(N / o.x1_bdiv) * Cout * Ho * Wo);
    nograd = pair;
  }
  for (int which = 0; which < 2; ++which) {
    const int ci = which ? c1 : c0;
    if (!ci) continue;
    Op::PackSlot& dg = o.dgrad[which];
    dg.geo = as_bf(conv2_choose(ks, 1, N, o.H, o.W, ci, Cout, (!o.ps && o.stride == 1) ? ks_ok : ALLOW_NONE), o.H, o.W, ci, true);
    dg.floats = conv2_pack_floats(ks, ci, Cout, dg.geo);
    dg.off = p.dpack_floats;
    p.dpack_floats += dg.floats * p.wsets;
  }
}

struct Builder {
  dvsr_edvr_plan& p;
  int pcur = 0;
  explicit Builder(dvsr_edvr_plan& plan) : p(plan) {}

  T alloc(const char* name, size_t numel) { return arena_alloc(p, name, numel); }
  static T view(const T& base, size_t off, size_t numel) {
    T t = base;
    t.off += off;
    t.numel = numel;
    return t;
  }
  struct CP { int w, b; };
  CP take() { CP c{pcur, pcur + 1}; pcur += 2; return c; }

  T conv(const char* name, CP cp, T x0, int c0, T x1, int c1, int N, int H, int W, int Cout, int ks,
         int stride, int act, T res = T(), int ps = 0, int x1_bdiv = 1, long long x0_bs = 0,
         long long x1_bs = 0, T y_override = T(), int pad = -1, int wmap = 0) {
    Op o;
    o.type = OP_CONV; o.name = name; o.pw = cp.w; o.pb = cp.b; o.pad = pad; o.wmap = wmap;
    o.x0 = x0; o.x1 = x1; o.res = res;
    o.N = N; o.c0 = c0; o.c1 = c1; o.H = H; o.W = W; o.Cout = Cout; o.ks = ks; o.stride = stride;
    o.act = act; o.ps = ps; o.x1_bdiv = x1_bdiv; o.x0_bs = x0_bs; o.x1_bs = x1_bs;
    o.y = y_override.valid() ? y_override : alloc(name, (size_t)N * Cout * conv_out(o, H) * conv_out(o, W));
    if (wmap) o.w2_off = alloc("", (size_t)std::max(p.wgroups, p.wsets) * Cout * (c0 + c1) * ks * ks).off;
    plan_conv_launches(o, p);
    p.ops.push_back(o);
    return o.y;
  }
  T dcn(const char* name, int pw, int pb, T x, T om, int N, int C, int H, int W, int dg, int act) {
    Op o;
    o.type = OP_DCN; o.name = name; o.pw = pw; o.pb = pb; o.x0 = x; o.x1 = om;
    o.N = N; o.c0 = C; o.H = H; o.W = W; o.Cout = C; o.dg = dg; o.act = act;
    o.y = alloc(name, (size_t)N * C * H * W);
    if (C % (dg * 8) == 0) {
      o.dcn_pack.floats = conv2_pack_floats(3, C, C, 8, 0, PackLayout::DCN_SPLIT);
      o.dcn_pack.off = alloc("", o.dcn_pack.floats * p.wsets).off;
    }
    p.ops.push_back(o);
    return o.y;
  }
  T up(const char* name, T x, size_t planes, int H, int W, int S, float mul) {
    Op o;
    o.type = OP_UP; o.name = name; o.x0 = x; o.planes = planes; o.H = H; o.W = W; o.S = S; o.mul = mul;
    o.y = alloc(name, planes * H * W * S * S);
    p.ops.push_back(o);
    return o.y;
  }
  T padop(const char* name, T x, int mode, int N, int C, int H, int W, int Tn) {
    Op o;
    o.type = OP_PAD; o.name = name; o.x0 = x; o.pmode = mode; o.N = N; o.c0 = C; o.H = H; o.W = W; o.T = Tn;
    o.y = alloc(name, pad_out_numel(mode, (size_t)N, C, H, W));
    p.ops.push_back(o);
    return o.y;
  }
  void pool(const char* name, T x, size_t planes, int H, int W, T& ymax, T& yavg) {
    Op o;
    o.type = OP_POOL; o.name = name; o.x0 = x; o.planes = planes; o.H = H; o.W = W;
    const size_t n = planes * (size_t)((H - 1) / 2 + 1) * ((W - 1) / 2 + 1);
    o.y = ymax = alloc((std::string(name) + "_max").c_str(), n);
    o.y2 = yavg = alloc((std::string(name) + "_avg").c_str(), n);
    p.ops.push_back(o);
  }
};

enum PlanPart { PART_WHOLE = 0, PART_EXTRACT = 1, PART_FUSE = 2 };

struct SlotLayout { size_t off[3], numel[3], raw, floats; };
static SlotLayout slot_layout(int C, int H, int W) {
  auto up = [](size_t n) { return (n + 63) & ~(size_t)63; };
  SlotLayout s;
  s.numel[0] = (size_t)C * H * W; s.numel[1] = (size_t)C * (H / 2) * (W / 2); s.numel[2] = (size_t)C * (H / 4) * (W / 4);
  s.off[0] = 0; s.off[1] = up(s.numel[0]); s.off[2] = s.off[1] + up(s.numel[1]);
  s.raw = s.off[2] + up(s.numel[2]);
  s.floats = s.raw + up((size_t)3 * H * W);
  return s;
}

static int build_plan(dvsr_edvr_plan& p, PlanPart part = PART_WHOLE) {
  const dvsr_edvr_config& c = p.cfg;
  const int B = p.B, Nf = c.nframes, C = c.nf, H = p.H, W = p.W, BN = B * Nf, dg = c.groups;
  const int H2 = H / 2, W2 = W / 2, H4 = H / 4, W4 = W / 4;
  const size_t HW = (size_t)H * W, HW2 = (size_t)H2 * W2, HW4 = (size_t)H4 * W4;
  Builder b(p);
  const int L = ACT_LRELU, R = ACT_RELU, NO = ACT_NONE;
  T none;
  const int EN = part == PART_EXTRACT ? 1 : BN;
  T xin; xin.space = SP_INPUT; xin.off = 0; xin.numel = (size_t)EN * 3 * HW;

  T f1, f2, f3;
  if (part == PART_FUSE) {
    f1 = b.alloc("L1_fea", (size_t)BN * C * HW);
    f2 = b.alloc("L2_fea", (size_t)BN * C * HW2);
    f3 = b.alloc("L3_fea", (size_t)BN * C * HW4);
    b.pcur += 2 * (1 + 2 * c.front_RBs + 4);
  } else {
    const SlotLayout sl = slot_layout(C, H, W);
    auto dst = [&](int l, bool final_of_level) {
      T t;
      if (part == PART_EXTRACT && final_of_level) { t.space = SP_OUTPUT; t.off = sl.off[l]; t.numel = sl.numel[l]; }
      return t;
    };
    f1 = b.conv("conv_first", b.take(), xin, 3, none, 0, EN, H, W, C, 3, 1, L, none, 0, 1, 0, 0, dst(0, c.front_RBs == 0));
    for (int i = 0; i < c.front_RBs; ++i) {
      auto p1 = b.take(); auto p2 = b.take();
      T t = b.conv("fe_rb_a", p1, f1, C, none, 0, EN, H, W, C, 3, 1, R);
      f1 = b.conv("fe_rb_b", p2, t, C, none, 0, EN, H, W, C, 3, 1, NO, f1, 0, 1, 0, 0, dst(0, i == c.front_RBs - 1));
    }
    p.named.emplace_back("L1_fea", f1);
    f2 = b.conv("fea_L2_conv1", b.take(), f1, C, none, 0, EN, H, W, C, 3, 2, L);
    f2 = b.conv("L2_fea", b.take(), f2, C, none, 0, EN, H2, W2, C, 3, 1, L, none, 0, 1, 0, 0, dst(1, true));
    f3 = b.conv("fea_L3_conv1", b.take(), f2, C, none, 0, EN, H2, W2, C, 3, 2, L);
    f3 = b.conv("L3_fea", b.take(), f3, C, none, 0, EN, H4, W4, C, 3, 1, L, none, 0, 1, 0, 0, dst(2, true));
  }
  if (part == PART_EXTRACT) {
    p.n_params = b.pcur;
    return DVSR_OK;
  }

  struct DP { int w, b; Builder::CP com; };
  auto take_dcn = [&]() { DP d; d.w = b.pcur; d.b = b.pcur + 1; b.pcur += 2; d.com = b.take(); return d; };
  auto L3o1 = b.take(); auto L3o2 = b.take(); DP L3d = take_dcn();
  auto L2o1 = b.take(); auto L2o2 = b.take(); auto L2o3 = b.take(); DP L2d = take_dcn(); auto L2f = b.take();
  auto L1o1 = b.take(); auto L1o2 = b.take(); auto L1o3 = b.take(); DP L1d = take_dcn(); auto L1f = b.take();
  auto cso1 = b.take(); auto cso2 = b.take(); DP csd = take_dcn();
  const int ctr = c.center;
  T ref1 = Builder::view(f1, (size_t)ctr * C * HW, 0), ref2 = Builder::view(f2, (size_t)ctr * C * HW2, 0),
    ref3 = Builder::view(f3, (size_t)ctr * C * HW4, 0);
  const long long rs1 = (long long)Nf * C * HW, rs2 = (long long)Nf * C * HW2, rs3 = (long long)Nf * C * HW4;
  T o3 = b.conv("L3_offset_conv1", L3o1, f3, C, ref3, C, BN, H4, W4, C, 3, 1, L, none, 0, Nf, 0, rs3);
  o3 = b.conv("L3_offset", L3o2, o3, C, none, 0, BN, H4, W4, C, 3, 1, L);
  T om3 = b.conv("L3_om", L3d.com, o3, C, none, 0, BN, H4, W4, dg * 27, 3, 1, NO);
  T fe3 = b.dcn("L3_aligned", L3d.w, L3d.b, f3, om3, BN, C, H4, W4, dg, L);
  T o2 = b.conv("L2_offset_conv1", L2o1, f2, C, ref2, C, BN, H2, W2, C, 3, 1, L, none, 0, Nf, 0, rs2);
  T u3 = b.up("L3_offset_up", o3, (size_t)BN * C, H4, W4, 2, 2.f);
  o2 = b.conv("L2_offset_conv2", L2o2, o2, C, u3, C, BN, H2, W2, C, 3, 1, L);
// ... 712 lines not shown
  static const int fork_env = [] { const char* v = getenv("DVSR_BWD_FORK_EVERY"); return v ? atoi(v) : 0; }();
  const int fork_every = fork_env > 0 ? fork_env : p->fork_every;
  std::vector<WgradLaunch> waiting;
  int waiting_layers = 0;
  auto flush_waiting = [&]() -> int {
    if (waiting.empty()) return DVSR_OK;
    hipStream_t ws = st;
    if (use_side) {
      DVSR_REQUIRE(hipEventRecord(p->ev_fork, st) == hipSuccess && hipStreamWaitEvent(p->side, p->ev_fork, 0) == hipSuccess,
                   DVSR_ERR_HIP, "edvr_backward: fork to the wgrad stream failed");
      ws = p->side;
      forked = true;
    }
    for (const WgradLaunch& l : waiting) {
      int rc = conv2d_wgrad_launch(l, ws);
      if (rc != DVSR_OK) return rc;
    }
    waiting.clear();
    waiting_layers = 0;
    return DVSR_OK;
  };
  for (const BOp& b : p->bops) {
    int rc = DVSR_OK;
    if (b.type == B_WGRAD) {
      reduces.emplace_back();
      WgradLaunch l;
      rc = prep_wgrad(*p, b, grad_params, bs, (char*)wscratch + b.ws_off, b.ws_bytes, st, &reduces.back(), &l);
      if (rc != DVSR_OK) return rc;
      if (b.fwd != last_fork_fwd) {
        if (waiting_layers >= fork_every) rc = flush_waiting();
        last_fork_fwd = b.fwd;
        ++waiting_layers;
      }
      waiting.push_back(l);
      if (rc == DVSR_OK && (!use_side || !l.geo.row_split)) rc = flush_waiting();
    } else if (b.type == B_WUNMAP) {
      unmaps.push_back(&b);
    } else {
      rc = run_backward_op(*p, b, params, grad_params, bs, scratch, p->scratch_bytes, st);
    }
    if (rc != DVSR_OK) return rc;
  }
  {
    int rc = flush_waiting();
    if (rc != DVSR_OK) return rc;
    hipStream_t ws = use_side && forked ? p->side : st;
    rc = wgrad_reduce_batch(reduces.data(), (int)reduces.size(), ws);
    if (rc != DVSR_OK) return rc;
    for (const BOp* b : unmaps) {
      rc = run_backward_op(*p, *b, params, grad_params, bs, nullptr, 0, ws);
      if (rc != DVSR_OK) return rc;
    }
  }
  if (forked)
    DVSR_REQUIRE(hipEventRecord(p->ev_join, p->side) == hipSuccess &&
                     hipStreamWaitEvent(st, p->ev_join, 0) == hipSuccess,
                 DVSR_ERR_HIP, "edvr_backward: join of the wgrad stream failed");
  return DVSR_OK;
}

extern "C" int dvsr_edvr_num_backward_launches(const dvsr_edvr_plan* p) { return p ? (int)p->bops.size() : -1; }

static FwdMode forward_mode(const dvsr_edvr_plan* p, size_t ws_bytes) {
  return ws_bytes < dvsr_edvr_workspace_bytes(p, 1) ? FWD_NOGRAD : FWD_GRAD;
}

static int run_forward_tape(const dvsr_edvr_plan& p, const float* const* params, const Bases& bs, bool packs_valid, hipStream_t st) {
  if (!p.use_v1 && !packs_valid) {
    int rc = pack_all(p, params, bs.arena, bs.arena, nullptr, st, bs.mode);
    if (rc != DVSR_OK) return rc;
  }
  for (const Op& o : p.ops) {
    int rc = run_forward_op(p, o, params, bs, st);
    if (rc != DVSR_OK) return rc;
  }
  return DVSR_OK;
}

static int edvr_forward_impl(const dvsr_edvr_plan* p, const float* const* params, const float* x, float* out, void* ws,
                             size_t ws_bytes, dvsr_stream_t stream, bool packs_valid);

extern "C" int dvsr_edvr_forward(const dvsr_edvr_plan* p, const float* const* params, const float* x,
                                 float* out, void* ws, size_t ws_bytes, dvsr_stream_t stream) {
  return edvr_forward_impl(p, params, x, out, ws, ws_bytes, stream, false);
}

extern "C" int dvsr_edvr_forward_packed(const dvsr_edvr_plan* p, const float* const* params, const float* x,
                                        float* out, void* ws, size_t ws_bytes, dvsr_stream_t stream) {
  return edvr_forward_impl(p, params, x, out, ws, ws_bytes, stream, true);
}

static int edvr_forward_impl(const dvsr_edvr_plan* p, const float* const* params, const float* x, float* out, void* ws,
                             size_t ws_bytes, dvsr_stream_t stream, bool packs_valid) {
  DVSR_REQUIRE(p && params && x && out && ws, DVSR_ERR_INVALID, "edvr_forward: null argument");
  DVSR_REQUIRE(ws_bytes >= p->arena_floats * sizeof(float), DVSR_ERR_WORKSPACE,
               "edvr_forward: workspace %zu < %zu bytes", ws_bytes, p->arena_floats * sizeof(float));
  return run_forward_tape(*p, params, Bases{(float*)ws, x, out, forward_mode(p, ws_bytes)}, packs_valid, (hipStream_t)stream);
}

static void op_work(const Op& o, const char** kind, double* flops, double* bytes) {
  *flops = 0; *bytes = 0; *kind = "other";
  switch (o.type) {
    case OP_CONV: {
      const int Ho = conv_out(o, o.H), Wo = conv_out(o, o.W);
      const double ctot = o.c0 + o.c1, px = (double)o.N * Ho * Wo;
      *flops = 2.0 * px * o.Cout * ctot * o.ks * o.ks;
      *bytes = 4.0 * ((double)o.N * o.c0 * o.H * o.W + (double)(o.N / o.x1_bdiv) * o.c1 * o.H * o.W +
                      px * o.Cout * (o.res.valid() ? 2 : 1) + (double)o.Cout * ctot * o.ks * o.ks);
      *kind = o.ks == 1 ? "conv1x1" : (o.ks == 2 ? "conv2x2" : (o.stride == 2 ? "conv3x3s2" : "conv3x3s1"));
      break;
    }
    case OP_DCN: {
      const double px = (double)o.N * o.H * o.W;
      *flops = 2.0 * px * o.Cout * o.c0 * 9 + px * o.c0 * 9 * 8.0;
      *bytes = 4.0 * (px * o.c0 + px * o.dg * 27 + px * o.Cout + (double)o.Cout * o.c0 * 9);
      *kind = "mdcn";
      break;
    }
    case OP_UP: *bytes = 4.0 * o.planes * o.H * o.W * (1.0 + o.S * o.S); *kind = "upsample"; break;
    case OP_POOL: *bytes = 4.0 * o.planes * o.H * o.W * 1.5; *kind = "pool"; break;
    case OP_GATE: *bytes = 4.0 * ((double)o.gB * o.gN * o.gC * o.gHW * 3 + (double)o.gB * o.gC * o.gHW +
                                 (double)o.gB * o.gN * o.gHW); *kind = "tsa_gate"; break;
    case OP_BLEND: *bytes = 4.0 * o.y.numel * 4; *kind = "tsa_blend"; break;
    case OP_ADD: *bytes = 4.0 * o.y.numel * 3; *kind = "add"; break;
    case OP_PAD: *bytes = 4.0 * ((double)o.N * o.c0 * o.H * o.W + (double)o.y.numel); *kind = "pad"; break;
    case OP_MEANSUB: *bytes = 4.0 * o.y.numel * 3; *kind = "meansub"; break;
    case OP_ADDMEAN: *bytes = 4.0 * o.y.numel * 2; *kind = "addmean"; break;
  }
}

extern "C" int dvsr_edvr_op_info(const dvsr_edvr_plan* p, int index, char* kind, int kind_cap,
                                 char* name, int name_cap, double* flops, double* bytes) {
  DVSR_REQUIRE(p && kind && name && flops && bytes && index >= 0 && index < (int)p->ops.size(),
               DVSR_ERR_INVALID, "edvr_op_info: bad argument");
  const char* k;
  op_work(p->ops[index], &k, flops, bytes);
  snprintf(kind, kind_cap, "%s", k);
  if (p->ops[index].type == OP_CONV)
  {
    const ConvGeo& g = p->ops[index].launches[FWD_NOGRAD].primary().pack.geo;
    snprintf(name, name_cap, "%s[%d/%d/%d%s]", p->ops[index].name, g.cc, g.th, g.mt, kernel_tag(g.kernel));
  }
  else
    snprintf(name, name_cap, "%s", p->ops[index].name);
  return DVSR_OK;
}

extern "C" int dvsr_edvr_op_launch_count(const dvsr_edvr_plan* p, int index, int nograd) {
  if (!p || index < 0 || index >= (int)p->ops.size()) return -1;
  const Op& o = p->ops[index];
  return o.type == OP_CONV ? o.launches[nograd ? FWD_NOGRAD : FWD_GRAD].n : 1;
}

static int plan_work(const dvsr_edvr_plan* p, double* out9, FwdMode mode) {
  DVSR_REQUIRE(p && out9, DVSR_ERR_INVALID, "edvr_plan_work: null argument");
  double fa = 0, fe = 0, ba = 0, be = 0, fby = 0, f32p[2] = {0, 0}, bfp[2] = {0, 0};
  auto conv_part = [](const Op& o, int ci) {
    return 2.0 * (double)o.N * conv_out(o, o.H) * conv_out(o, o.W) * o.Cout * ci * o.ks * o.ks;
  };
  auto issue = [&](const ConvGeo& g, double f, double* ex, int pass) {
    const double shaped = f * multiplies_per_output_ratio(g.kernel);
    *ex += shaped;
    if (on_bf16_split(g.kernel) || g.bf == 2) bfp[pass] += 6.0 * shaped;
    else if (g.bf == 1) bfp[pass] += shaped;
    else f32p[pass] += shaped;
  };
  for (const Op& o : p->ops) {
    {
      const char* k; double fl, by;
      op_work(o, &k, &fl, &by);
      fby += by;
    }
    if (o.type == OP_CONV) {
      const double f = conv_part(o, o.c0 + o.c1);
      fa += f;
      for (const Op::Launch& l : o.launches[mode])
        issue(l.pack.geo, conv_part(o, l.c) / (l.role == Op::REF_PART ? o.x1_bdiv : 1), &fe, 0);
    } else if (o.type == OP_DCN) {
      const double f = 2.0 * (double)o.N * o.H * o.W * o.Cout * o.c0 * 9;
      fa += f; fe += f; f32p[0] += f;
    }
  }
  for (const BOp& b : p->bops) {
    if (b.fwd < 0) continue;
    const Op& o = p->ops[b.fwd];
    if (b.type == B_WGRAD) {
      const double f = conv_part(o, b.which ? o.c1 : o.c0);
      ba += f; be += f;
      const WgradKernel k = conv2d_wgrad_choose(wgrad_shape(*p, o, b.which)).kernel;
      if (on_bf16_split(k)) bfp[1] += 6.0 * f; else if (on_bf16_pipe(k)) bfp[1] += f; else f32p[1] += f;
    } else if (b.type == B_DGRAD) {
      const double f = conv_part(o, b.which ? o.c1 : o.c0);
      ba += f; issue(o.dgrad[b.which].geo, f, &be, 1);
    } else if (b.type == B_DCN) {
      const double f = 2.0 * 2.0 * (double)o.N * o.H * o.W * o.Cout * o.c0 * 9;
      ba += f; be += f; f32p[1] += f;
    }
  }
  out9[0] = fa; out9[1] = fe; out9[2] = ba; out9[3] = be;
  out9[4] = fby;
  out9[5] = f32p[0]; out9[6] = bfp[0]; out9[7] = f32p[1]; out9[8] = bfp[1];
  return DVSR_OK;
}
extern "C" int dvsr_edvr_plan_work(const dvsr_edvr_plan* p, double* out9) { return plan_work(p, out9, FWD_GRAD); }
extern "C" int dvsr_edvr_plan_work_nograd(const dvsr_edvr_plan* p, double* out9) { return plan_work(p, out9, FWD_NOGRAD); }

extern "C" int dvsr_edvr_forward_timed(const dvsr_edvr_plan* p, const float* const* params,
                                       const float* x, float* out, void* ws, size_t ws_bytes,
                                       dvsr_stream_t stream, float* op_ms) {
  DVSR_REQUIRE(p && params && x && out && ws && op_ms, DVSR_ERR_INVALID, "edvr_forward_timed: null argument");
  DVSR_REQUIRE(ws_bytes >= p->arena_floats * sizeof(float), DVSR_ERR_WORKSPACE,
               "edvr_forward_timed: workspace too small");
  hipStream_t st = (hipStream_t)stream;
  const size_t n = p->ops.size();
  std::vector<hipEvent_t> ev(n + 1);
  for (auto& e : ev) DVSR_REQUIRE(hipEventCreate(&e) == hipSuccess, DVSR_ERR_HIP, "hipEventCreate failed");
  const Bases bs{(float*)ws, x, out, forward_mode(p, ws_bytes)};
  int rc = p->use_v1 ? DVSR_OK : pack_all(*p, params, bs.arena, bs.arena, nullptr, st, bs.mode);
  hipEventRecord(ev[0], st);
  for (size_t i = 0; i < n && rc == DVSR_OK; ++i) {
    rc = run_forward_op(*p, p->ops[i], params, bs, st);
    hipEventRecord(ev[i + 1], st);
  }
  if (rc == DVSR_OK && hipStreamSynchronize(st) != hipSuccess) {
    set_error("edvr_forward_timed: stream synchronize failed");
    rc = DVSR_ERR_HIP;
  }
  if (rc == DVSR_OK)
    for (size_t i = 0; i < n; ++i) hipEventElapsedTime(&op_ms[i], ev[i], ev[i + 1]);
  for (auto& e : ev) hipEventDestroy(e);
  return rc;
}

extern "C" int dvsr_edvr_op_output(const dvsr_edvr_plan* p, int index, int which, int* in_arena, long long* offset_floats,
                                   long long* numel) {
  DVSR_REQUIRE(p && in_arena && offset_floats && numel && index >= 0 && index < (int)p->ops.size() && (which == 0 || which == 1),
               DVSR_ERR_INVALID, "edvr_op_output: bad argument");
  const T& t = which ? p->ops[index].y2 : p->ops[index].y;
  DVSR_REQUIRE(t.valid(), DVSR_ERR_INVALID, "edvr_op_output: launch %d has no output %d", index, which);
  *in_arena = t.space == SP_ARENA;
  *offset_floats = (long long)t.off;
  *numel = (long long)t.numel;
  return DVSR_OK;
}

extern "C" int dvsr_edvr_tensor_info(const dvsr_edvr_plan* p, const char* name, long long* offset_floats,
                                     long long* numel) {
  DVSR_REQUIRE(p && name && offset_floats && numel, DVSR_ERR_INVALID, "edvr_tensor_info: null argument");
  for (const auto& kv : p->named)
    if (kv.first == name && kv.second.space == SP_ARENA) {
      *offset_floats = (long long)kv.second.off;
      *numel = (long long)kv.second.numel;
      return DVSR_OK;
    }
  set_error("edvr_tensor_info: no tensor named '%s'", name);
  return DVSR_ERR_INVALID;
}


struct dvsr_edvr_stream {
  dvsr_edvr_plan extract, fuse;
  int slots = 0;
  dvsr::SlotLayout sl;
  size_t fea_off[3] = {0, 0, 0};
};

extern "C" int dvsr_edvr_stream_create(const dvsr_edvr_config* cfg, int H, int W, int slots, dvsr_edvr_stream** out) {
  DVSR_REQUIRE(cfg && out, DVSR_ERR_INVALID, "edvr_stream_create: null argument");
  DVSR_REQUIRE(H > 0 && W > 0 && H % 4 == 0 && W % 4 == 0, DVSR_ERR_INVALID,
               "edvr_stream_create: H=%d W=%d (H, W must be positive multiples of 4)", H, W);
  DVSR_REQUIRE(cfg->nf > 0 && cfg->groups > 0 && cfg->nf % cfg->groups == 0 && cfg->nframes > 0 && cfg->front_RBs >= 0 &&
                   cfg->back_RBs >= 0, DVSR_ERR_INVALID, "edvr_stream_create: bad network config");
  DVSR_REQUIRE(cfg->nframes <= DVSR_STREAM_MAX_FRAMES, DVSR_ERR_UNSUPPORTED, "edvr_stream_create: nframes=%d (at most %d)",
               cfg->nframes, DVSR_STREAM_MAX_FRAMES);
  DVSR_REQUIRE(slots >= cfg->nframes, DVSR_ERR_INVALID, "edvr_stream_create: slots=%d < nframes=%d", slots, cfg->nframes);
  DVSR_REQUIRE(cfg->scale == 4 || cfg->scale == 2, DVSR_ERR_UNSUPPORTED, "edvr_stream_create: scale=%d (2 or 4)", cfg->scale);
  DVSR_REQUIRE(cfg->center >= 0 && cfg->center < cfg->nframes, DVSR_ERR_INVALID, "edvr_stream_create: center=%d out of range",
               cfg->center);
  const int cpg = cfg->nf / cfg->groups;
  DVSR_REQUIRE(cpg == 4 || cpg == 8 || cpg == 16, DVSR_ERR_UNSUPPORTED, "edvr_stream_create: nf/groups=%d (supported: 4, 8, 16)", cpg);
  dvsr_edvr_stream* s = new dvsr_edvr_stream();
  const char* v1 = getenv("DVSR_CONV_V1");
  int k = 0;
  for (dvsr_edvr_plan* p : {&s->extract, &s->fuse}) {
    p->cfg = *cfg; p->B = 1; p->H = H; p->W = W;
    p->use_v1 = v1 && v1[0] == '1';
    int rc = build_plan(*p, k++ == 0 ? PART_EXTRACT : PART_FUSE);
    if (rc != DVSR_OK) { delete s; return rc; }
  }
  s->slots = slots;
  s->sl = slot_layout(cfg->nf, H, W);
  static const char* const names[3] = {"L1_fea", "L2_fea", "L3_fea"};
  for (int l = 0; l < 3; ++l)
    for (const auto& kv : s->fuse.named)
      if (kv.first == names[l]) s->fea_off[l] = kv.second.off;
  *out = s;
  return DVSR_OK;
}

extern "C" void dvsr_edvr_stream_destroy(dvsr_edvr_stream* s) { delete s; }

extern "C" int dvsr_edvr_stream_num_params(const dvsr_edvr_stream* s) { return s ? s->fuse.n_params : -1; }

extern "C" int dvsr_edvr_stream_num_launches(const dvsr_edvr_stream* s, int which) {
  if (!s) return -1;
  return which ? (int)s->fuse.ops.size() + 1 : (int)s->extract.ops.size();
// ... 300 lines not shown
```

### dynavsr_amd/csrc/kernels.h

```cpp
#pragma once
#include "../../include/dynavsr_hip.h"
#include "common.h"

namespace dvsr {

struct ConvExtra {
  int wt = 0;
  int w_ctot = 0, w_coff = 0;
  int in_ps = 0;
  int in_dil = 0, Hs = 0, Ws = 0;
  int accum = 0;
  const float* gmask = nullptr;
  int gmask_act = 0;
  int wdiv = 1; long long w_gs = 0; int b_gs = 0;
};
int conv2d_run(const dvsr_conv2d_desc& d, const ConvExtra& ex, hipStream_t st);

int mdcn_forward_run(const float* x, const float* off, long long off_bs, const float* msk,
                     long long msk_bs, int mask_logit, const float* w, const float* b, float* out,
                     int N, int C, int H, int W, int Cout, int kh, int kw, int stride, int pad,
                     int dil, int groups, int dg, int act, hipStream_t st);

enum class ConvKernel : int {
  REG = 0,
  DMA_HALO = 1,
  ROW_SPLIT = 2,
  WINO_F2 = 3,
  WINO_F2_BF16 = 4,
  WINO_F4 = 5,
};
enum class PackLayout : int {
  INTERLEAVED = 0,
  DMA_ORDER = 1,
  ROW_SPLIT = 2,
  WINO_F2 = 3,
  WINO_F2_BF16 = 4,
  WINO_F4 = 5,
  DCN_SPLIT = 6,
};
constexpr PackLayout pack_layout(ConvKernel k) { return static_cast<PackLayout>(static_cast<int>(k)); }
constexpr bool is_winograd(ConvKernel k) { return k == ConvKernel::WINO_F2 || k == ConvKernel::WINO_F2_BF16 || k == ConvKernel::WINO_F4; }
constexpr bool on_bf16_split(ConvKernel k) { return k == ConvKernel::WINO_F2_BF16 || k == ConvKernel::WINO_F4; }
constexpr bool needs_dma_halo_inputs(ConvKernel k) { return k == ConvKernel::DMA_HALO || is_winograd(k); }
constexpr double multiplies_per_output_ratio(ConvKernel k) { return k == ConvKernel::WINO_F4 ? 0.25 : (is_winograd(k) ? 16.0 / 36.0 : 1.0); }
constexpr const char* kernel_tag(ConvKernel k) {
  return k == ConvKernel::WINO_F4 ? "w5" : (k == ConvKernel::WINO_F2_BF16 ? "w3" : (k == ConvKernel::WINO_F2 ? "w" : (k == ConvKernel::REG ? "" : "d")));
}
constexpr bool has_own_pack_kernel(PackLayout l) { return static_cast<int>(l) >= static_cast<int>(PackLayout::WINO_F2); }

struct PackEntry {
  const float* w; float* P;
  int Cout, Ctot, KK, CC, wt, w_ctot, w_coff, ncb, nchunks, pch;
  int bf = 0;
  PackLayout layout = PackLayout::INTERLEAVED;
};
struct PackTable {
  int n;
  PackEntry e[48];
};
int pack_weights_run(const PackTable& t, hipStream_t st);
struct ConvGeo { int cc, th, mt; int bf = 0; ConvKernel kernel = ConvKernel::REG; };
enum ConvAllow : int {
  ALLOW_NONE = 0,
  ALLOW_KSPLIT = 1,
  ALLOW_DMA_HALO = 2,
  ALLOW_WINO = 4,
  ALLOW_WINO_F4 = 8,
  ALLOW_SHARED_DEVICE = 16,
  ALLOW_ONLY_F4 = 32,
};
constexpr ConvAllow operator|(ConvAllow a, ConvAllow b) { return static_cast<ConvAllow>(static_cast<int>(a) | static_cast<int>(b)); }
constexpr ConvAllow without(ConvAllow a, ConvAllow b) { return static_cast<ConvAllow>(static_cast<int>(a) & ~static_cast<int>(b)); }
ConvGeo conv2_choose(int ks, int stride, int N, int Ho, int Wo, int Cout, int Ctot, ConvAllow allow = ALLOW_KSPLIT);
size_t conv2_pack_floats(int ks, int Cout, int Ctot, int cc, int bf, PackLayout layout);
PackEntry conv2_pack_entry(const float* w, float* P, int ks, int Cout, int Ctot, int cc, int bf, PackLayout layout, int wt = 0,
                           int w_ctot = 0, int w_coff = 0);
inline size_t conv2_pack_floats(int ks, int Cout, int Ctot, const ConvGeo& g) {
  return conv2_pack_floats(ks, Cout, Ctot, g.cc, g.bf, pack_layout(g.kernel));
}
inline PackEntry conv2_pack_entry(const float* w, float* P, int ks, int Cout, int Ctot, const ConvGeo& g, int wt = 0, int w_ctot = 0,
                                  int w_coff = 0) {
  return conv2_pack_entry(w, P, ks, Cout, Ctot, g.cc, g.bf, pack_layout(g.kernel), wt, w_ctot, w_coff);
}
double conv2_f4_occupied_cycles(int N, int Ho, int Wo, int Cout, int Ctot, int th);
int pack_weights_wino_run(const PackTable& t, hipStream_t st);
int pack_weights_wino3_run(const PackTable& t, hipStream_t st);
int pack_weights_wino5_run(const PackTable& t, hipStream_t st);
int conv2d_packed_run(const dvsr_conv2d_desc& d, const float* wp, const ConvExtra& ex, const ConvGeo& geo,
                      hipStream_t st);

bool conv1x1_dual_ok(const float* x, const float* w0, const float* w1, const float* y0, const float* y1, int Cin, long long HW);
int conv1x1_dual_run(const float* x, const float* w0, const float* b0, const float* w1, const float* b1, float* y0, float* y1,
                     int N, int Cin, int HW, int act, hipStream_t st, int wdiv = 1, long long w_gs = 0, int b_gs = 0);
int conv3x3_small_cout_run(const float* x, const float* w, const float* bias, const float* res, float* y, int N,
                           int C, int H, int W, int Cout, int act, hipStream_t st, int wdiv = 1, long long w_gs = 0,
                           int b_gs = 0);

struct WgradReduceEntry {
  float* partial; float* dbp; float* dW; float* db;
  int nslot, KK, OP, CP, Cout, Cin, Ctot, c_off;
  int ngroups = 1;
  long long dW_gs = 0, db_gs = 0;
};
constexpr int WGRAD_REDUCE_BATCH = 44;
struct WgradReduceTable {
  int n;
  WgradReduceEntry e[WGRAD_REDUCE_BATCH];
};
int wgrad_reduce_batch(const WgradReduceEntry* entries, int n, hipStream_t st, int blocks = 96);
struct WgradDesc {
  const float* x = nullptr; long long x_bs = 0; int x_bdiv = 1;
  const float* gy = nullptr; int gy_ps = 0;
  float* dW = nullptr; float* db = nullptr;
  int N = 0, Cin = 0, H = 0, W = 0, Cout = 0, Ctot = 0, c_off = 0, ks = 0, stride = 1, pad = -1;
  int groups = 1; long long dW_gs = 0, db_gs = 0;
  int mode = 0;
};
enum class WgradKernel : int {
  SIMPLE = 0,
  PIPE = 1,
  BF16 = 2,
  SPLIT_SCALAR = 3,
  SPLIT_VECTOR = 4,
  SPLIT_WAVE8 = 5,
};
constexpr bool on_bf16_pipe(WgradKernel k) { return k >= WgradKernel::BF16; }
constexpr bool on_bf16_split(WgradKernel k) { return k >= WgradKernel::SPLIT_SCALAR; }
struct WgradGeo {
  WgradKernel kernel = WgradKernel::PIPE;
  int row_split = 0;
  int vx = 0;
  int nsplit = 1, nslot = 1;
  dim3 grid; int block = 256;
};
WgradGeo conv2d_wgrad_choose(const WgradDesc& d);
bool wgrad_split3_default();
size_t conv2d_wgrad_workspace_bytes(const WgradDesc& d);
int conv2d_wgrad_run(const WgradDesc& d, void* ws, size_t ws_bytes, hipStream_t st, int scratch_is_zero = 0,
                     WgradReduceEntry* defer = nullptr);
size_t mdcn_backward_workspace_bytes(int N, int C, int H, int W, int Cout, int stride, int pad, int dil, int groups = 1);
int mdcn_backward_run(const float* x, const float* off, long long off_bs, const float* msk, long long msk_bs,
                      int mask_logit, const float* w, const float* gout, float* gx, float* goff,
                      long long goff_bs, float* gmsk, long long gmsk_bs, float* gw, float* gb, int N, int C,
                      int H, int W, int Cout, int stride, int pad, int dil, int dg, void* ws,
                      size_t ws_bytes, hipStream_t st, int groups = 1, long long gw_gs = 0, long long gb_gs = 0,
                      long long w_gs = 0);

int mdcn_forward_packed_run(const float* x, const float* off, long long off_bs, const float* msk,
                            long long msk_bs, int mask_logit, const float* wp, const float* b, float* out,
                            int N, int C, int H, int W, int Cout, int dg, int act, hipStream_t st, int wdiv = 1,
                            long long w_gs = 0, int b_gs = 0, PackLayout layout = PackLayout::INTERLEAVED);
int mdcn_fwd_variant();
int mdcn_pack_floats();
PackLayout mdcn_pack_layout(int W);
int pack_weights_dcn3_run(const PackTable& t, hipStream_t st);

struct DcnK2 {
  const float* x; const float* off; const float* msk; const float* wp; const float* bias; float* out;
  long long off_bstride, msk_bstride;
  int mask_logit;
  int N, C, H, W, Cout, dg, act;
  int tiles_x, tiles_y, ntiles, ncb, nchunks;
  int wdiv = 1; long long w_gs = 0; int b_gs = 0;
#ifdef DVSR_CONV_TRACE
  long long* trace;
#endif
};
int mdcn_fwd_split_launch(const DcnK2& k, int grid, int mask_logit, hipStream_t st);

int upsample_bilinear_fwd(const float* x, float* y, size_t planes, int H, int W, int S, float mul,
                          hipStream_t st);
int upsample_bilinear_bwd(const float* gy, float* gx, size_t planes, int H, int W, int S, float mul,
                          int accumulate, hipStream_t st);
int pool3s2_fwd(const float* x, float* ymax, float* yavg, size_t planes, int H, int W, hipStream_t st);
int pool3s2_bwd(const float* x, const float* gmax, const float* gavg, float* gx, size_t planes,
                int H, int W, int accumulate, hipStream_t st);
int reduce_frames(float* dst, long long dst_bs, const float* src, int B, int cnt, size_t per,
                  int accumulate, hipStream_t st);
int tsa_gate_fwd(const float* emb, const float* emb_ref, const float* aligned, float* cor,
                 float* gated, int B, int N, int C, size_t HW, hipStream_t st);
int tsa_gate_bwd(const float* emb, const float* emb_ref, const float* aligned, const float* cor,
                 const float* g_gated, float* g_emb, float* g_emb_ref, float* g_aligned, int B,
                 int N, int C, size_t HW, hipStream_t st, float* gdot_scratch = nullptr);
int tsa_blend_fwd(const float* fea, const float* att, const float* add, float* out, size_t n,
                  hipStream_t st);
int tsa_blend_bwd(const float* fea, const float* att, const float* g, float* g_fea, float* g_att_io,
                  size_t n, int accumulate, hipStream_t st);
int add_inplace(float* dst, const float* src, size_t n, hipStream_t st);
int add_out(float* y, const float* a, const float* b, size_t n, hipStream_t st);
int act_bwd_inplace(float* g, const float* y, size_t n, int act, hipStream_t st);

int stream_gather_run(const float* cache, size_t slot_floats, const size_t src_off[3], float* const dst[3],
                      const size_t level_floats[3], int nframes, const int* slots, hipStream_t st);

hipStream_t side_stream_for(hipStream_t st, bool* known = nullptr);

int frame_ingest_check(const char* what, const void* src, const dvsr_frame_desc* sd, const float* dst, int Hp, int Wp,
                       int pad_mode);
int frame_ingest_launch(const void* src, const dvsr_frame_desc& sd, float* dst, int Hp, int Wp, int pad_mode, hipStream_t st);

struct YuvFrame {
  void* plane[3];
  long long rs[3];
  int h, w, matrix, range;
  bool semi;
  int bytes, depth;
  int chroma;
};
int yuv_frame_from(const char* what, const dvsr_yuv_desc* d, YuvFrame* f);
int yuv_frame_from(const char* what, const dvsr_yuv16_desc* d, YuvFrame* f);
int frame_ingest_yuv_check(const char* what, const YuvFrame& f, const float* dst, int Hp, int Wp, int pad_mode);
int frame_ingest_yuv_launch(const YuvFrame& f, float* dst, int Hp, int Wp, int pad_mode, hipStream_t st);

enum : int { PAD_REFLECT = 0, PAD_REFLECT_S2D = 1, PAD_REPL_T3 = 2 };
size_t pad_out_numel(int mode, size_t N, int C, int H, int W);
int pad_fwd(const float* x, float* y, int mode, int N, int C, int H, int W, int T, hipStream_t st);
int pad_bwd(const float* gy, float* gx, int mode, int N, int C, int H, int W, int T, int accumulate,
            hipStream_t st, const float* gmask = nullptr, int gmask_act = 0, int gmask_padded = 0);
int meansub_slices();
int meansub_fwd(const float* x, float* xm, float* mean, float* part, int B, int C, int T, int H, int W,
                hipStream_t st);
int addmean_fwd(const float* y, const float* mean, float* out, int B, int C, int T, size_t HW, hipStream_t st);
int addmean_bwd(const float* gout, float* gy, int B, int C, int T, size_t HW, hipStream_t st);
int w4_to_s2d(const float* w, float* w2, int Cout, int C, int inverse, hipStream_t st);

__device__ __forceinline__ float sigmoidf_(float v) { return 1.f / (1.f + expf(-v)); }

struct DcnTap {
  int o1, o2, o3, o4;
  float w1, w2, w3, w4;
  float lh, lw;
  bool v1, v2, v3, v4;
};

__device__ __forceinline__ bool make_tap(float h_im, float w_im, int H, int W, DcnTap& t) {
  if (!(h_im > -1.f && w_im > -1.f && h_im < (float)H && w_im < (float)W)) return false;
  const int h_lo = (int)floorf(h_im), w_lo = (int)floorf(w_im);
  const int h_hi = h_lo + 1, w_hi = w_lo + 1;
  t.lh = h_im - (float)h_lo;
  t.lw = w_im - (float)w_lo;
  const float hh = 1.f - t.lh, hw = 1.f - t.lw;
  t.v1 = h_lo >= 0 && w_lo >= 0;
// ... 13 lines not shown
```

### dynavsr_amd/engine.py

```python
import ctypes
import threading

import torch

from . import _lib as L

_plans = {}
_GEOMETRY_ENV = ("DVSR_CONV_WINO", "DVSR_CONV_WINO3", "DVSR_CONV_WINO5", "DVSR_CONV_V1", "DVSR_EST_SPLIT", "DVSR_EST_SPLIT2", "DVSR_FUSE_ACT_BWD",
                 "DVSR_BWD_STREAMS", "DVSR_PCD_HOIST")
_PROCESS_ENV = ("DVSR_CONV_LDS", "DVSR_CONV_LAST_MFMA", "DVSR_SPLIT_TH8_FROM", "DVSR_WGRAD_SPLIT3",
                "DVSR_WGRAD_WIDE", "DVSR_WGRAD_S3V", "DVSR_WGRAD_S3_KYS_BELOW", "DVSR_WGRAD_S3_WGS", "DVSR_WGRAD_S3W", "DVSR_DCN_FWD", "DVSR_DCN_BWD",
                "DVSR_EST_FUSE_PAD", "DVSR_FUSE_RES_BWD", "DVSR_BWD_FORK_EVERY", "DVSR_BWD_PROBE", "DVSR_TSA_DUAL", "DVSR_TSA_V",
                "DVSR_DEGRADE_GENERIC", "DVSR_UP2")
_process_env_seen = None


def _check_process_env():
    import os
    import warnings
    global _process_env_seen
    now = tuple(os.environ.get(k) for k in _PROCESS_ENV)
    if _process_env_seen is None:
        _process_env_seen = now
        return
    for k, a, b in zip(_PROCESS_ENV, _process_env_seen, now):
        if a != b:
            warnings.warn("dynavsr_amd: %s=%r now, but the native library read %r when the first plan of this process was built "
                          "and keeps that value (switches of this kind are read once per process: set them before the first "
                          "plan, one process per value)" % (k, b, a), RuntimeWarning, stacklevel=3)
    _process_env_seen = now


_WORK_KEYS = ("fwd_algorithmic", "fwd_executed", "bwd_algorithmic", "bwd_executed", "fwd_bytes",
              "fwd_f32_pipe", "fwd_bf16_pipe", "bwd_f32_pipe", "bwd_bf16_pipe")


def _env_key():
    import os
    return tuple(os.environ.get(k) for k in _GEOMETRY_ENV)


class Plan:

    def __init__(self, cfg, b, h, w, grad_groups=1, weight_sets=1):
        self.key = (cfg, b, h, w, grad_groups, weight_sets)
        cfg = tuple(cfg) + (0,) * (8 - len(cfg))
        self.cfg = dict(zip(("nf", "nframes", "groups", "front_RBs", "back_RBs", "scale", "center", "bf16_mfma"), cfg))
        self.b, self.h, self.w, self.grad_groups, self.weight_sets = b, h, w, grad_groups, weight_sets
        self._h = ctypes.c_void_p()
        L.check(L.lib().dvsr_edvr_plan_create_ex(L.EdvrConfig(*cfg), b, h, w, grad_groups, weight_sets,
                                                 ctypes.byref(self._h)), "dvsr_edvr_plan_create_ex")
        self.n_params = L.lib().dvsr_edvr_num_params(self._h)
        self.n_launches = L.lib().dvsr_edvr_num_launches(self._h)
        self.n_backward_launches = L.lib().dvsr_edvr_num_backward_launches(self._h)

    def workspace_bytes(self, need_grad):
        return int(L.lib().dvsr_edvr_workspace_bytes(self._h, int(need_grad)))

    def forward(self, params, x, out, ws, packed=False):
        arr = (ctypes.c_void_p * len(params))(*[L.ptr(p) for p in params])
        fn = L.lib().dvsr_edvr_forward_packed if packed else L.lib().dvsr_edvr_forward
        L.check(fn(self._h, arr, L.ptr(x), L.ptr(out), ws.data_ptr(), ws.numel() * ws.element_size(), L.stream()),
                "dvsr_edvr_forward_packed" if packed else "dvsr_edvr_forward")

    def backward(self, params, x, gout, gparams, gx, ws):
        arr = (ctypes.c_void_p * len(params))(*[L.ptr(p) for p in params])
        garr = (ctypes.c_void_p * len(gparams))(*[L.ptr(g) for g in gparams])
        L.check(L.lib().dvsr_edvr_backward(self._h, arr, L.ptr(x), L.ptr(gout), garr, L.ptr(gx),
                                           ws.data_ptr(), ws.numel() * ws.element_size(), L.stream()),
                "dvsr_edvr_backward")

    def forward_timed(self, params, x, out, ws):
        arr = (ctypes.c_void_p * len(params))(*[L.ptr(p) for p in params])
        ms = (ctypes.c_float * self.n_launches)()
        L.check(L.lib().dvsr_edvr_forward_timed(self._h, arr, L.ptr(x), L.ptr(out), ws.data_ptr(),
                                                ws.numel() * ws.element_size(), L.stream(), ms),
                "dvsr_edvr_forward_timed")
        return list(ms)

    def work(self, nograd=False):
        out = (ctypes.c_double * 9)()
        fn = L.lib().dvsr_edvr_plan_work_nograd if nograd else L.lib().dvsr_edvr_plan_work
        L.check(fn(self._h, ctypes.byref(out)), "dvsr_edvr_plan_work")
        return dict(zip(_WORK_KEYS, out))

    def op_output(self, ws, index, which=0):
        ia, off, n = ctypes.c_int(), ctypes.c_longlong(), ctypes.c_longlong()
        L.check(L.lib().dvsr_edvr_op_output(self._h, index, which, ctypes.byref(ia), ctypes.byref(off), ctypes.byref(n)),
                "dvsr_edvr_op_output")
        if not ia.value:
            return None
        return ws.view(torch.float32)[off.value:off.value + n.value]

    def op_info(self):
        out = []
        kind, name = ctypes.create_string_buffer(32), ctypes.create_string_buffer(64)
        fl, by = ctypes.c_double(), ctypes.c_double()
        for i in range(self.n_launches):
            L.check(L.lib().dvsr_edvr_op_info(self._h, i, kind, 32, name, 64, ctypes.byref(fl),
                                              ctypes.byref(by)), "dvsr_edvr_op_info")
            out.append((kind.value.decode(), name.value.decode(), fl.value, by.value))
        return out

    def tensor(self, ws, name, shape=None):
        off, n = ctypes.c_longlong(), ctypes.c_longlong()
        L.check(L.lib().dvsr_edvr_tensor_info(self._h, name.encode(), ctypes.byref(off),
                                              ctypes.byref(n)), "dvsr_edvr_tensor_info")
        t = ws.view(torch.float32)[off.value:off.value + n.value]
        return t.view(shape) if shape is not None else t

    def __del__(self):
        try:
            if self._h:
                L.lib().dvsr_edvr_plan_destroy(self._h)
        except Exception:
            pass


def get_plan(cfg, b, h, w, device=None, grad_groups=1, weight_sets=1):
    dev = torch.cuda.current_device() if device is None else torch.device(device).index
    key = (tuple(cfg), b, h, w, dev, torch.cuda.current_stream(dev).cuda_stream, grad_groups, weight_sets, _env_key())
    p = _plans.get(key)
    if p is None:
        _check_process_env()
        p = _plans[key] = Plan(tuple(cfg), b, h, w, grad_groups, weight_sets)
    return p


def _stash(ctx, plan, ws, x, params):
    ctx.plan, ctx.ws, ctx.x, ctx.params = plan, ws, x, params
    ctx.versions = [p._version for p in params]


def _check_stash(ctx, what):
    if ctx.ws is None:
        raise RuntimeError("%s: backward called a second time -- the activation arena was released after the "
                           "first one (the tape is first-order and single-use, like once_differentiable in "
                           "deform_conv.py:123)" % what)
    for i, (p, v) in enumerate(zip(ctx.params, ctx.versions)):
        if p._version != v:
            raise RuntimeError("%s: parameter %d was modified in place between forward and backward (version %d -> "
                               "%d); the gradient would be taken at the wrong weights" % (what, i, v, p._version))


def _prep(t):
    if t.dtype != torch.float32:
        t = t.float()
    return t.contiguous()


_grad_mode = threading.local()


class _TapeFunction(torch.autograd.Function):

    @classmethod
    def apply(cls, *args, **kwargs):
        _grad_mode.enabled = torch.is_grad_enabled()
        return super().apply(*args, **kwargs)


def _need_grad(ctx):
# ... 371 lines not shown
```

### include/dynavsr_hip.h

```cpp
#ifndef DYNAVSR_HIP_H_
#define DYNAVSR_HIP_H_

#include <stddef.h>

#ifdef __cplusplus
extern "C" {
#endif

#define DVSR_OK 0
#define DVSR_ERR_INVALID (-1)
#define DVSR_ERR_UNSUPPORTED (-2)
#define DVSR_ERR_WORKSPACE (-3)
#define DVSR_ERR_HIP (-4)

#define DVSR_ACT_NONE 0
#define DVSR_ACT_LRELU 1
#define DVSR_ACT_RELU 2

typedef void* dvsr_stream_t;

const char* dvsr_last_error(void);
int dvsr_version(void);

int dvsr_mdcn_forward(const float* x, const float* offset, const float* mask, const float* w,
                      const float* b, float* out, int N, int C, int H, int W, int Cout, int kh,
                      int kw, int stride, int pad, int dil, int groups, int dg, int act,
                      dvsr_stream_t stream);

size_t dvsr_mdcn_forward_fast_workspace_bytes(int C, int Cout, int dg);
int dvsr_mdcn_forward_fast(const float* x, const float* offset, const float* mask, const float* w,
                           const float* b, float* out, int N, int C, int H, int W, int Cout, int dg, int act,
                           void* workspace, size_t workspace_bytes, dvsr_stream_t stream);

size_t dvsr_mdcn_backward_workspace_bytes(int N, int C, int H, int W, int Cout, int kh, int kw, int stride,
                                          int pad, int dil);
int dvsr_mdcn_backward(const float* x, const float* offset, const float* mask, const float* w,
                       const float* grad_out, float* gx, float* goffset, float* gmask, float* gw, float* gb,
                       int N, int C, int H, int W, int Cout, int kh, int kw, int stride, int pad, int dil,
                       int groups, int dg, void* workspace, size_t workspace_bytes, dvsr_stream_t stream);

int dvsr_mdcn_pack_forward(const float* x, const float* om, const float* w, const float* b,
                           float* out, int N, int C, int H, int W, int Cout, int kh, int kw,
                           int stride, int pad, int dil, int groups, int dg, int act,
                           dvsr_stream_t stream);

int dvsr_mdcn_pack_forward_fast(const float* x, const float* om, const float* w, const float* b, float* out, int N,
                                int C, int H, int W, int Cout, int dg, int act, void* workspace,
                                size_t workspace_bytes, dvsr_stream_t stream);

typedef struct dvsr_conv2d_desc {
  const float* x0;
  const float* x1;
  const float* w;
  const float* bias;
  const float* res;
  float* y;
  int N, c0, c1, H, W, Cout;
  int ks;
  int stride;
  int pad;
  int act;
  int pixel_shuffle;
  int x1_bdiv;
  long long x0_bstride;
  long long x1_bstride;
  const float* pre;
  int pre_bdiv;
} dvsr_conv2d_desc;

int dvsr_conv2d_forward(const dvsr_conv2d_desc* d, dvsr_stream_t stream);
size_t dvsr_conv2d_backward_workspace_bytes(const dvsr_conv2d_desc* d);
int dvsr_conv2d_backward(const dvsr_conv2d_desc* d, const float* gy, float* gx0, float* gx1, float* gw,
                         float* gb, void* workspace, size_t workspace_bytes, dvsr_stream_t stream);

int dvsr_upsample_bilinear_forward(const float* x, float* y, long long planes, int H, int W,
                                   int scale, float mul, dvsr_stream_t stream);
int dvsr_upsample_bilinear_backward(const float* gy, float* gx, long long planes, int H, int W,
                                    int scale, float mul, int accumulate, dvsr_stream_t stream);
int dvsr_pool3s2_forward(const float* x, float* ymax, float* yavg, long long planes, int H, int W,
                         dvsr_stream_t stream);
int dvsr_pool3s2_backward(const float* x, const float* gmax, const float* gavg, float* gx,
                          long long planes, int H, int W, dvsr_stream_t stream);
int dvsr_tsa_gate_forward(const float* emb, const float* emb_ref, const float* aligned, float* cor,
                          float* gated, int B, int N, int C, long long HW, dvsr_stream_t stream);
int dvsr_tsa_gate_backward(const float* emb, const float* emb_ref, const float* aligned,
                           const float* cor, const float* g_gated, float* g_emb, float* g_emb_ref,
                           float* g_aligned, int B, int N, int C, long long HW,
                           dvsr_stream_t stream);
int dvsr_tsa_blend_forward(const float* fea, const float* att, const float* att_add, float* out,
                           long long n, dvsr_stream_t stream);
int dvsr_tsa_blend_backward(const float* fea, const float* att, const float* g, float* g_fea,
                            float* g_att_io, long long n, dvsr_stream_t stream);

typedef struct dvsr_edvr_config {
  int nf, nframes, groups, front_RBs, back_RBs, scale, center;
  int bf16_mfma;
} dvsr_edvr_config;
typedef struct dvsr_edvr_plan dvsr_edvr_plan;

int dvsr_edvr_plan_create(const dvsr_edvr_config* cfg, int B, int H, int W, dvsr_edvr_plan** out);
int dvsr_edvr_plan_create_grouped(const dvsr_edvr_config* cfg, int B, int H, int W, int grad_groups,
                                  dvsr_edvr_plan** out);
int dvsr_edvr_plan_create_ex(const dvsr_edvr_config* cfg, int B, int H, int W, int grad_groups, int weight_sets,
                             dvsr_edvr_plan** out);
void dvsr_edvr_plan_destroy(dvsr_edvr_plan* plan);
int dvsr_edvr_num_params(const dvsr_edvr_plan* plan);
int dvsr_edvr_num_launches(const dvsr_edvr_plan* plan);
size_t dvsr_edvr_workspace_bytes(const dvsr_edvr_plan* plan, int need_grad);
int dvsr_edvr_forward(const dvsr_edvr_plan* plan, const float* const* params, const float* x,
                      float* out, void* workspace, size_t workspace_bytes, dvsr_stream_t stream);
int dvsr_edvr_forward_packed(const dvsr_edvr_plan* plan, const float* const* params, const float* x,
                             float* out, void* workspace, size_t workspace_bytes, dvsr_stream_t stream);
int dvsr_edvr_backward(const dvsr_edvr_plan* plan, const float* const* params, const float* x,
                       const float* grad_out, float* const* grad_params, float* grad_x, void* workspace,
                       size_t workspace_bytes, dvsr_stream_t stream);
int dvsr_edvr_num_backward_launches(const dvsr_edvr_plan* plan);
int dvsr_edvr_op_info(const dvsr_edvr_plan* plan, int index, char* kind, int kind_cap, char* name,
                      int name_cap, double* flops, double* bytes);
int dvsr_edvr_plan_work(const dvsr_edvr_plan* plan, double* out9);
int dvsr_edvr_plan_work_nograd(const dvsr_edvr_plan* plan, double* out9);
int dvsr_edvr_op_launch_count(const dvsr_edvr_plan* plan, int index, int nograd);
int dvsr_side_stream_overlaps(dvsr_stream_t stream);
int dvsr_edvr_op_output(const dvsr_edvr_plan* plan, int index, int which, int* in_arena, long long* offset_floats,
                        long long* numel);
int dvsr_edvr_forward_timed(const dvsr_edvr_plan* plan, const float* const* params, const float* x,
                            float* out, void* workspace, size_t workspace_bytes,
                            dvsr_stream_t stream, float* op_ms);
long long dvsr_debug_mfma_peak(float* out, int blocks, int iters, int nacc, int lds_bytes, dvsr_stream_t stream);
int dvsr_debug_mfma_shadow(long long* cycles, float* out, int blocks, int iters, int nv, int kind, int acc,
                           dvsr_stream_t stream);
int dvsr_edvr_tensor_info(const dvsr_edvr_plan* plan, const char* name, long long* offset_floats,
                          long long* numel);

#define DVSR_STREAM_MAX_FRAMES 16
typedef struct dvsr_edvr_stream dvsr_edvr_stream;
int dvsr_edvr_stream_create(const dvsr_edvr_config* cfg, int H, int W, int slots, dvsr_edvr_stream** out);
void dvsr_edvr_stream_destroy(dvsr_edvr_stream* stream_plan);
int dvsr_edvr_stream_num_params(const dvsr_edvr_stream* stream_plan);
int dvsr_edvr_stream_num_launches(const dvsr_edvr_stream* stream_plan, int which);
size_t dvsr_edvr_stream_cache_bytes(const dvsr_edvr_stream* stream_plan);
size_t dvsr_edvr_stream_workspace_bytes(const dvsr_edvr_stream* stream_plan);
unsigned long long dvsr_edvr_stream_max_image_bytes(const dvsr_edvr_stream* stream_plan);
int dvsr_edvr_stream_extract(const dvsr_edvr_stream* stream_plan, const float* const* params, const float* frame, int slot,
                             void* cache, size_t cache_bytes, void* workspace, size_t workspace_bytes, int packed,
                             dvsr_stream_t stream);
int dvsr_edvr_stream_fuse(const dvsr_edvr_stream* stream_plan, const float* const* params, const int* slots,
                          const void* cache, size_t cache_bytes, float* out, void* workspace, size_t workspace_bytes,
                          int packed, dvsr_stream_t stream);

#define DVSR_FRAME_F32_CHW 0
#define DVSR_FRAME_U8_HWC_RGB 1
#define DVSR_FRAME_U8_HWC_BGR 2
#define DVSR_FRAME_PAD_REFLECT 0
#define DVSR_FRAME_PAD_REPLICATE 1
typedef struct dvsr_frame_desc {
  int format;
  int h, w;
  long long row_stride, plane_stride;
  int pixel_stride;
} dvsr_frame_desc;
int dvsr_frame_ingest(const void* src, const dvsr_frame_desc* sd, float* dst, int Hp, int Wp, int pad_mode,
                      dvsr_stream_t stream);
int dvsr_frame_emit(const float* src, int Hs, int Ws, void* dst, const dvsr_frame_desc* dd, float lo, float hi,
                    dvsr_stream_t stream);
int dvsr_edvr_stream_extract_frame(const dvsr_edvr_stream* stream_plan, const float* const* params, const void* frame,
                                   const dvsr_frame_desc* fd, int pad_mode, int slot, void* cache, size_t cache_bytes,
                                   void* workspace, size_t workspace_bytes, int packed, dvsr_stream_t stream);

#define DVSR_FRAME_U8_Y 3
#define DVSR_FRAME_U16_Y_MSB 4
#define DVSR_FRAME_U16_Y_10 5
#define DVSR_FRAME_U16_Y_12 6
int dvsr_frame_luma_sad(const void* a, const void* b, const dvsr_frame_desc* desc, long long frame_stride, int pairs,
                        unsigned long long* sad, dvsr_stream_t stream);

#define DVSR_YUV_NV12 0
#define DVSR_YUV_I420 1
#define DVSR_YUV_CHROMA_420 0
#define DVSR_YUV_CHROMA_422 1
#define DVSR_YUV_CHROMA_444 2
#define DVSR_YUV_FORMAT(form, chroma) ((form) | ((chroma) << 4))
#define DVSR_YUV_BT601 0
#define DVSR_YUV_BT709 1
#define DVSR_YUV_LIMITED 0
#define DVSR_YUV_FULL 1
typedef struct dvsr_yuv_desc {
  int format;
  int h, w;
  int matrix, range;
  void* plane[3];
  long long row_stride[3];
} dvsr_yuv_desc;
int dvsr_frame_ingest_yuv(const dvsr_yuv_desc* sd, float* dst, int Hp, int Wp, int pad_mode, dvsr_stream_t stream);
int dvsr_frame_emit_yuv(const float* src, int Hs, int Ws, const dvsr_yuv_desc* dd, float lo, float hi, dvsr_stream_t stream);
int dvsr_edvr_stream_extract_frame_yuv(const dvsr_edvr_stream* stream_plan, const float* const* params, const dvsr_yuv_desc* fd,
                                       int pad_mode, int slot, void* cache, size_t cache_bytes, void* workspace,
                                       size_t workspace_bytes, int packed, dvsr_stream_t stream);

#define DVSR_YUV16_SEMI_MSB 0
#define DVSR_YUV16_PLANAR_LSB 1
typedef struct dvsr_yuv16_desc {
  int format, depth;
  int h, w;
  int matrix, range;
  void* plane[3];
  long long row_stride[3];
} dvsr_yuv16_desc;
int dvsr_frame_ingest_yuv16(const dvsr_yuv16_desc* sd, float* dst, int Hp, int Wp, int pad_mode, dvsr_stream_t stream);
int dvsr_frame_emit_yuv16(const float* src, int Hs, int Ws, const dvsr_yuv16_desc* dd, float lo, float hi, dvsr_stream_t stream);
int dvsr_edvr_stream_extract_frame_yuv16(const dvsr_edvr_stream* stream_plan, const float* const* params,
                                         const dvsr_yuv16_desc* fd, int pad_mode, int slot, void* cache, size_t cache_bytes,
                                         void* workspace, size_t workspace_bytes, int packed, dvsr_stream_t stream);

typedef struct dvsr_resize_axis {
  const int* first;
  const float* weights;
  int taps;
} dvsr_resize_axis;
int dvsr_frame_resize_taps(int n_in, int n_out);
int dvsr_frame_resize_table(int n_in, int n_out, int taps, int* first, float* weights);
int dvsr_frame_resize(const float* src, int Hs, int Ws, int h, int w, float* dst, int Ho, int Wo, int oh, int ow,
                      const dvsr_resize_axis* rows, const dvsr_resize_axis* cols, dvsr_stream_t stream);

#define DVSR_FLIP_W 1
#define DVSR_FLIP_H 2
int dvsr_frame_flip(const float* src, float* dst, long long planes, int H, int W, int flags, dvsr_stream_t stream);
int dvsr_frame_flip_mean(const float* y0, const float* yw, const float* yh, const float* yhw, float* dst,
                         long long planes, int H, int W, dvsr_stream_t stream);

typedef struct dvsr_stitch_axis {
  const int* first;
  const float* weights;
  const int* origins;
  int cover;
} dvsr_stitch_axis;
int dvsr_frame_stitch_origins(int n, int tile, int overlap, int* origins, int capacity);
int dvsr_frame_stitch_cover(int n, int tile, int overlap);
int dvsr_frame_stitch_table(int n, int tile, int overlap, int scale, int cover, int* first, float* weights);
int dvsr_frame_stitch(const float* tiles, int ny, int nx, int planes, int Ht, int Wt, float* dst, int H, int W,
                      const dvsr_stitch_axis* rows, const dvsr_stitch_axis* cols, const int* origins_y, const int* origins_x,
                      dvsr_stream_t stream);

#define DVSR_ESTIMATOR_MFDN 0
#define DVSR_ESTIMATOR_SFDN 1
typedef struct dvsr_estimator_config {
  int kind;
  int nf;
  int in_nc;
  int scale;
  int nframes;
} dvsr_estimator_config;
typedef struct dvsr_estimator_plan dvsr_estimator_plan;
int dvsr_estimator_plan_create(const dvsr_estimator_config* cfg, int B, int H, int W, dvsr_estimator_plan** out);
int dvsr_estimator_plan_create_grouped(const dvsr_estimator_config* cfg, int B, int H, int W, int grad_groups,
                                       dvsr_estimator_plan** out);
int dvsr_estimator_plan_create_ex(const dvsr_estimator_config* cfg, int B, int H, int W, int grad_groups, int weight_sets,
                                  dvsr_estimator_plan** out);
void dvsr_estimator_plan_destroy(dvsr_estimator_plan* plan);
int dvsr_estimator_num_params(const dvsr_estimator_plan* plan);
int dvsr_estimator_num_launches(const dvsr_estimator_plan* plan, int backward);
int dvsr_estimator_plan_work(const dvsr_estimator_plan* plan, double* out9);
size_t dvsr_estimator_workspace_bytes(const dvsr_estimator_plan* plan, int need_grad);
int dvsr_estimator_forward(const dvsr_estimator_plan* plan, const float* const* params, const float* x, float* out,
                           void* workspace, size_t workspace_bytes, dvsr_stream_t stream);
int dvsr_estimator_backward(const dvsr_estimator_plan* plan, const float* const* params, const float* x,
                            const float* grad_out, float* const* grad_params, void* workspace,
                            size_t workspace_bytes, dvsr_stream_t stream);

size_t dvsr_charbonnier_workspace_bytes(void);
int dvsr_charbonnier_forward(const float* x, const float* y, float* loss, long long n, float eps,
                             void* workspace, size_t workspace_bytes, dvsr_stream_t stream);
int dvsr_charbonnier_backward(const float* x, const float* y, const float* grad_loss, float* gx, long long n,
                              float eps, dvsr_stream_t stream);
int dvsr_charbonnier_forward_grouped(const float* x, const float* y, float* loss, long long n, int groups, float eps,
                                     void* workspace, size_t workspace_bytes, dvsr_stream_t stream);
int dvsr_charbonnier_backward_grouped(const float* x, const float* y, const float* grad_loss, float* gx, long long n,
                                      int groups, float eps, dvsr_stream_t stream);

int dvsr_l1_tail_forward(const float* x, const float* y, const float* base, float weight, float* loss, long long n,
                         void* workspace, size_t workspace_bytes, dvsr_stream_t stream);
int dvsr_l1_tail_backward(const float* x, const float* y, const float* grad_loss, float weight, float* gx, long long n,
                          dvsr_stream_t stream);
int dvsr_l1_tail_forward_grouped(const float* x, const float* y, const float* base, float weight, float* loss, long long n,
                                 int groups, void* workspace, size_t workspace_bytes, dvsr_stream_t stream);
int dvsr_l1_tail_backward_grouped(const float* x, const float* y, const float* grad_loss, float weight, float* gx,
                                  long long n, int groups, dvsr_stream_t stream);

size_t dvsr_conv2d_packed_workspace_bytes(const dvsr_conv2d_desc* d);
int dvsr_conv2d_forward_packed(const dvsr_conv2d_desc* d, void* workspace, size_t workspace_bytes, dvsr_stream_t stream);
int dvsr_conv2d_dgrad_packed(const dvsr_conv2d_desc* d, const float* gy, float* gx0, void* workspace,
                             size_t workspace_bytes, dvsr_stream_t stream);
int dvsr_conv2d_packed_geometry(const dvsr_conv2d_desc* d, int geo[4]);

int dvsr_conv2d_wgrad_bf16(const dvsr_conv2d_desc* d, const float* gy, float* gw, float* gb, void* workspace,
                           size_t workspace_bytes, dvsr_stream_t stream);
int dvsr_conv2d_wgrad_split3(const dvsr_conv2d_desc* d, const float* gy, float* gw, float* gb, void* workspace,
                             size_t workspace_bytes, dvsr_stream_t stream);

int dvsr_conv2d_wgrad_geometry(const dvsr_conv2d_desc* d, int mode, int groups, int geo[8]);
size_t dvsr_conv2d_wgrad_workspace_bytes(const dvsr_conv2d_desc* d, int groups);

int dvsr_flow_warp_forward(const float* x, const float* flow, float* out, int N, int C, int H, int W,
                           long long out_bstride, dvsr_stream_t stream);
int dvsr_flow_warp_backward(const float* x, const float* flow, const float* grad_out, float* grad_x, float* grad_flow,
                            int N, int C, int H, int W, long long gout_bstride, dvsr_stream_t stream);
int dvsr_avgpool2_forward(const float* x, float* y, long long planes, int H, int W, dvsr_stream_t stream);
int dvsr_avgpool2_backward(const float* grad_y, float* grad_x, long long planes, int H, int W, int accumulate,
                           dvsr_stream_t stream);
int dvsr_resize_bilinear_ac_forward(const float* x, float* y, long long planes, int H, int W, int Ho, int Wo, float mul,
                                    long long y_plane_stride, dvsr_stream_t stream);
int dvsr_resize_bilinear_ac_backward(const float* grad_y, float* grad_x, long long planes, int H, int W, int Ho, int Wo,
                                     float mul, long long gy_plane_stride, dvsr_stream_t stream);
int dvsr_upsample_bicubic_ac_forward(const float* x, float* y, long long planes, int H, int W, int scale,
                                     dvsr_stream_t stream);
int dvsr_upsample_bicubic_ac_backward(const float* grad_y, float* grad_x, long long planes, int H, int W, int scale,
                                      dvsr_stream_t stream);
int dvsr_channel_affine(const float* x, const float* scale, const float* shift, float* out, int N, int C, long long HW,
                        long long x_bstride, long long out_bstride, int accumulate, dvsr_stream_t stream);
size_t dvsr_batchnorm_workspace_bytes(int C);
int dvsr_batchnorm_forward(const float* x, const float* gamma, const float* beta, float* running_mean,
                           float* running_var, float* y, float* save_mean, float* save_rstd, int N, int C, long long HW,
                           int training, float momentum, float eps, int relu, void* workspace, size_t workspace_bytes,
                           dvsr_stream_t stream);
int dvsr_batchnorm_backward(const float* x, const float* grad_y, const float* y, const float* gamma,
                            const float* save_mean, const float* save_rstd, float* grad_x, float* grad_gamma,
                            float* grad_beta, int N, int C, long long HW, int training, int relu, void* workspace,
                            size_t workspace_bytes, dvsr_stream_t stream);

int dvsr_temporal_gather3_forward(const float* x, float* y, int B, int T, int C, long long HW, int pad_t,
                                  dvsr_stream_t stream);
int dvsr_temporal_gather3_backward(const float* grad_y, float* grad_x, int B, int T, int C, long long HW, int pad_t,
                                   dvsr_stream_t stream);
int dvsr_dynamic_filter_forward(const float* x_center, const float* filter_logits, const float* residual, float* out,
                                int B, int H, int W, int scale, int adapt_official, dvsr_stream_t stream);
int dvsr_dynamic_filter_backward(const float* x_center, const float* filter_logits, const float* grad_out,
                                 float* grad_logits, float* grad_residual, float* grad_x_center, int B, int H, int W,
                                 int scale, int adapt_official, dvsr_stream_t stream);

int dvsr_conv3x3_small_cout(const float* x, const float* w, const float* bias, const float* res, float* y, int N, int C, int H,
                            int W, int Cout, int act, dvsr_stream_t stream);

int dvsr_conv1x1_dual(const float* x, const float* w0, const float* b0, const float* w1, const float* b1, float* y0, float* y1,
                      int N, int Cin, int H, int W, int act, dvsr_stream_t stream);

int dvsr_patch_gather_forward(const float* src, float* dst, const int* py, const int* px, int P, int planes, int H, int W,
                              int edge, int scale, dvsr_stream_t stream);
int dvsr_patch_gather_backward(const float* grad_dst, float* grad_src, const int* py, const int* px, int P, int planes,
                               int H, int W, int edge, int scale, dvsr_stream_t stream);

int dvsr_adam_step(float* const* params, const float* const* grads, float* const* exp_avg,
                   float* const* exp_avg_sq, const long long* numel, int n_tensors, float lr, float beta1,
                   float beta2, float eps, float weight_decay, int step, dvsr_stream_t stream);
int dvsr_sgd_step(float* const* params, const float* const* grads, const long long* numel, int n_tensors,
                  float lr, float weight_decay, dvsr_stream_t stream);
int dvsr_replicate_tensors(const float* const* src, float* const* dst, const long long* numel, int n_tensors, int copies,
                           dvsr_stream_t stream);

size_t dvsr_frame_metrics_workspace_bytes(int C, int H, int W);
int dvsr_frame_metrics(const float* sr, const float* gt, int C, int H, int W, float lo, float hi,
                       unsigned char* sr_hwc_u8, double* out, void* workspace, size_t workspace_bytes,
                       dvsr_stream_t stream);

#define DVSR_SCORE_RGB 0
#define DVSR_SCORE_Y 1
typedef struct dvsr_score_args {
  int channel;
  int crop_border, depth;
  float lo, hi;
} dvsr_score_args;
size_t dvsr_frame_score_workspace_bytes(int channels, int h, int w);
int dvsr_frame_score(const void* a, const dvsr_frame_desc* da, const void* b, const dvsr_frame_desc* db,
                     const dvsr_score_args* args, double* out , void* workspace,
                     size_t workspace_bytes, dvsr_stream_t stream);

int dvsr_degrade_apply(const float* img, const float* kernels, float* out, int N, int C, int H, int W, int K,
                       int scale, int n_kernels, int kernel_offset, int quantise, dvsr_stream_t stream);

#ifdef __cplusplus
}
#endif
#endif
```

Measured before the change: 259.4 frames/s.

## Add bf16x3-split MFMA kernel for 3x3 stride-2 convolutions

Adds a dedicated kernel for 3x3 stride-2 pad-1 convolutions. It splits each fp32 input into three bf16 pieces and runs bf16 32x32x16 MFMAs instead of the fp32 32x32x2 MFMA path. The kernel double-buffers weights via global_load_lds, stages input halos in LDS and uses an XCD-aware tile mapping. It is selected by default (DVSR_CONV_S2_SPLIT=1) for the no-grad forward of eligible PCD stride-2 convs, which adds a new packing path and a precision approximation of fp32 (three-term bf16 split). Ablation hooks are also added to the trace build of the existing kernel.

```diff
diff --git a/dynavsr_amd/_lib.py b/dynavsr_amd/_lib.py
--- a/dynavsr_amd/_lib.py
+++ b/dynavsr_amd/_lib.py
@@ -161,6 +161,7 @@
         "dvsr_conv2d_forward_packed": (I, [POINTER(Conv2dDesc), P, c_size_t, P]),
         "dvsr_conv2d_dgrad_packed": (I, [POINTER(Conv2dDesc), P, P, P, c_size_t, P]),
         "dvsr_conv2d_packed_geometry": (I, [POINTER(Conv2dDesc), POINTER(ctypes.c_int * 4)]),
+        "dvsr_conv2d_packed_pipe": (I, [POINTER(Conv2dDesc)]),
         "dvsr_conv2d_wgrad_geometry": (I, [POINTER(Conv2dDesc), I, I, POINTER(ctypes.c_int * 8)]),
         "dvsr_conv2d_wgrad_workspace_bytes": (c_size_t, [POINTER(Conv2dDesc), I]),
         "dvsr_conv2d_wgrad_bf16": (I, [POINTER(Conv2dDesc), P, P, P, P, c_size_t, P]),
@@ -201,6 +202,7 @@
         "dvsr_edvr_plan_work": (I, [P, POINTER(ctypes.c_double * 9)]),
         "dvsr_edvr_plan_work_nograd": (I, [P, POINTER(ctypes.c_double * 9)]),
         "dvsr_edvr_op_launch_count": (I, [P, I, I]),
+        "dvsr_edvr_op_matrix_pipe": (I, [P, I, I]),
         "dvsr_side_stream_overlaps": (I, [P]),
         "dvsr_edvr_op_output": (I, [P, I, I, POINTER(c_int), POINTER(LL), POINTER(LL)]),
         "dvsr_estimator_plan_work": (I, [P, POINTER(ctypes.c_double * 9)]),
diff --git a/dynavsr_amd/csrc/conv2d_s2split.hip b/dynavsr_amd/csrc/conv2d_s2split.hip
--- /dev/null
+++ b/dynavsr_amd/csrc/conv2d_s2split.hip
@@ -0,0 +1,243 @@
+#include <type_traits>
+
+#include "common.h"
+#include "kernels.h"
+#include "small_grid.h"
+
+namespace dvsr {
+
+typedef __bf16 s2bf8 __attribute__((ext_vector_type(8)));
+
+template <int MT>
+struct S2Shape {
+  static constexpr int TH = 4, IH = 9, HP = 33;
+  static constexpr int PAIRS = IH * HP;
+  static constexpr int E = (PAIRS + 255) / 256;
+  static constexpr int IN1 = IH * 2 * HP;
+  static constexpr int IN_F4 = 3 * IN1;
+  static constexpr int NHB = MT == 2 ? 2 : 1;
+  static constexpr int WROW = 32 * MT;
+  static constexpr int NROW = 27;
+  static constexpr int NDMA = MT == 2 ? 27 : 14;
+  static constexpr int W_F4 = NDMA * 64;
+  static constexpr int NWB = 2;
+  static constexpr size_t LDS_BYTES = (size_t)(NHB * IN_F4 + NWB * W_F4) * 16;
+};
+
+template <int MT, bool VEC2>
+__global__ __launch_bounds__(256, 2) void conv2d_s2split_kernel(ConvK2 a) {
+  using Sh = S2Shape<MT>;
+  constexpr int IH = Sh::IH, HP = Sh::HP, E = Sh::E, IN1 = Sh::IN1;
+  extern __shared__ __attribute__((aligned(16))) float smem[];
+  f32x4* const s_in0 = reinterpret_cast<f32x4*>(smem);
+  f32x4* const s_w0 = s_in0 + Sh::NHB * Sh::IN_F4;
+
+  const int id = blockIdx.x;
+  const int q_ = id >> 3;
+  const int cbi = q_ % a.ncb;
+  const int j_ = q_ / a.ncb;
+  const int tile = (id & 7) * a.tiles_per_xcd + j_;
+  if (j_ >= a.tiles_per_xcd || tile >= a.ntiles) return;
+  const int tx_ = tile % a.tiles_x;
+  const int t2 = tile / a.tiles_x;
+  const int ty_ = t2 % a.tiles_y;
+  const int n = t2 / a.tiles_y;
+  const int oy0 = ty_ * 4, ox0 = tx_ * 32;
+  const int iy0 = oy0 * 2 - 1, gx0 = ox0 * 2 - 2;
+
+  const int tid = threadIdx.x, lane = tid & 63;
+  const int wave = __builtin_amdgcn_readfirstlane(tid >> 6);
+  const int lo = lane & 31, hi = lane >> 5;
+  const size_t HW = (size_t)a.H * a.W;
+  const float* x0n = a.x0 + (size_t)n * a.x0_bs;
+
+  unsigned eoff[E][2];
+  bool va[E], vb[E], own[E];
+  int erec[E], ej[E];
+#pragma unroll
+  for (int e = 0; e < E; ++e) {
+    const int idx = tid + 256 * e;
+    const int iy = idx / HP, j = idx - iy * HP;
+    const int gy = iy0 + iy, gxa = gx0 + 2 * j;
+    own[e] = idx < Sh::PAIRS;
+    const bool row_ok = own[e] && (unsigned)gy < (unsigned)a.H;
+    va[e] = row_ok && (unsigned)gxa < (unsigned)a.W;
+    vb[e] = row_ok && (unsigned)(gxa + 1) < (unsigned)a.W;
+    const unsigned o = (unsigned)(gy * a.W + gxa) * 4u;
+    eoff[e][0] = va[e] ? o : 0u;
+    eoff[e][1] = vb[e] ? o + 4u : 0u;
+    erec[e] = (iy * 2) * HP + j;
+    ej[e] = j;
+  }
+
+  f32x16 acc[MT][1];
+#pragma unroll
+  for (int i = 0; i < MT; ++i)
+#pragma unroll
+    for (int r = 0; r < 16; ++r) acc[i][0][r] = 0.f;
+
+  const float* wp_cb = wset_ptr(a.wp, a.w_gs, n, a.wdiv) + (size_t)((cbi * MT) >> 1) * a.nchunks * 6912 + ((cbi * MT) & 1) * 128;
+
+  float ra[8][E], rb[8][E];
+  auto issue_halo = [&](int k) {
+    const char* p = reinterpret_cast<const char*>(x0n + (size_t)(k * 8) * HW);
+#pragma unroll
+    for (int c = 0; c < 8; ++c) {
+#pragma unroll
+      for (int e = 0; e < E; ++e) {
+        if (e == 0 || wave == 0) {
+          if constexpr (VEC2) {
+            const f32x2 v = *reinterpret_cast<const f32x2*>(p + eoff[e][0]);
+            ra[c][e] = v[0]; rb[c][e] = v[1];
+          } else {
+            ra[c][e] = *reinterpret_cast<const float*>(p + eoff[e][0]);
+            rb[c][e] = *reinterpret_cast<const float*>(p + eoff[e][1]);
+          }
+        }
+      }
+      p += HW * 4;
+    }
+  };
+  auto issue_w = [&](int k, int buf) {
+    const float* wsrc = wp_cb + (size_t)k * 6912;
+    f32x4* wdst = s_w0 + buf * Sh::W_F4;
+#pragma unroll
+    for (int j = 0; j < (Sh::NDMA + 3) / 4; ++j) {
+      int i = j * 4 + wave;
+      i = i < Sh::NDMA ? i : Sh::NDMA - 1;
+      const float* src;
+      if constexpr (MT == 2) {
+        src = wsrc + i * 256 + lane * 4;
+      } else {
+        int row = 2 * i + hi;
+        row = row < Sh::NROW ? row : Sh::NROW - 1;
+        src = wsrc + row * 256 + lo * 4;
+      }
+      __builtin_amdgcn_global_load_lds((const __attribute__((address_space(1))) void*)src,
+                                       (__attribute__((address_space(3))) void*)(wdst + i * 64), 16, 0, 0);
+    }
+  };
+  auto write_halo = [&](int buf) {
+    f32x4* s_in = s_in0 + buf * Sh::IN_F4;
+#pragma unroll
+    for (int e = 0; e < E; ++e) {
+      if (e == 0 || wave == 0) {
+#pragma unroll
+        for (int el = 0; el < 2; ++el) {
+          const bool ok = el ? vb[e] : va[e];
+          s2bf8 p0, p1, p2;
+#pragma unroll
+          for (int c = 0; c < 8; ++c) {
+            const float x = ok ? (el ? rb[c][e] : ra[c][e]) : 0.f;
+            const __bf16 h = (__bf16)x;
+            const float r1 = x - (float)h;
+            const __bf16 m = (__bf16)r1;
+            p0[c] = h; p1[c] = m; p2[c] = (__bf16)(r1 - (float)m);
+          }
+          if (own[e] && (el || ej[e] > 0)) {
+            f32x4* dst = s_in + erec[e] + (el ? 0 : HP - 1);
+            dst[0] = __builtin_bit_cast(f32x4, p0);
+            dst[IN1] = __builtin_bit_cast(f32x4, p1);
+            dst[2 * IN1] = __builtin_bit_cast(f32x4, p2);
+          }
+        }
+      }
+    }
+  };
+
+  const int b1 = ((hi ? 1 : 0) * IH + 2 * wave) * 2 * HP + lo, b2 = ((hi ? 2 : 0) * IH + 2 * wave) * 2 * HP + lo;
+  const int a1 = lo, a2 = (hi ? 0 : 1) * Sh::WROW + lo, a3 = (hi ? 1 : 2) * Sh::WROW + lo;
+
+  auto compute = [&](int k) {
+    const f32x4* s_in = s_in0 + (k % Sh::NHB) * Sh::IN_F4;
+    const f32x4* s_w = s_w0 + (k % Sh::NWB) * Sh::W_F4;
+    constexpr int AHEAD = MT == 1 ? 2 : 1;
+    f32x4 A[3][3][MT], B[3][2];
+    auto load_ops = [&](int tap, int rbuf) {
+      const int ty = tap / 3, tx = tap - ty * 3;
+      const int bo = (ty * 2 + (tx & 1)) * HP + (tx >> 1);
+      B[rbuf][0] = s_in[b1 + bo];
+      B[rbuf][1] = s_in[b2 + bo];
+#pragma unroll
+      for (int mt = 0; mt < MT; ++mt) {
+        const int ao = tap * 3 * Sh::WROW + mt * 32;
+        A[rbuf][2][mt] = s_w[a3 + ao];
+        A[rbuf][1][mt] = s_w[a2 + ao];
+        A[rbuf][0][mt] = s_w[a1 + ao];
+      }
+    };
+#pragma unroll
+    for (int t = 0; t < AHEAD; ++t) load_ops(t, t);
+    __builtin_amdgcn_sched_barrier(0);
+#pragma unroll
+    for (int tap = 0; tap < 9; ++tap) {
+      const int rbuf = tap % 3;
+      auto mm = [&](int pa, int pb) {
+#pragma unroll
+        for (int mt = 0; mt < MT; ++mt)
+          acc[mt][0] = __builtin_amdgcn_mfma_f32_32x32x16_bf16(__builtin_bit_cast(s2bf8, A[rbuf][pa][mt]),
+                                                               __builtin_bit_cast(s2bf8, B[rbuf][pb]), acc[mt][0], 0, 0, 0);
+      };
+      mm(2, 0);
+      __builtin_amdgcn_sched_barrier(0);
+      if (tap + AHEAD < 9) load_ops(tap + AHEAD, (tap + AHEAD) % 3);
+      __builtin_amdgcn_sched_barrier(0);
+      mm(1, 1);
+      mm(0, 0);
+      __builtin_amdgcn_sched_barrier(0);
+    }
+  };
+
+  auto drain_and_barrier = [&]() {
+    asm volatile("s_waitcnt vmcnt(0) lgkmcnt(0)" ::: "memory");
+    __builtin_amdgcn_s_barrier();
+    asm volatile("" ::: "memory");
+  };
+  issue_w(0, 0);
+  issue_halo(0);
+  write_halo(0);
+  drain_and_barrier();
+  for (int k = 0; k < a.nchunks; ++k) {
+    const bool has_next = k + 1 < a.nchunks;
+    if (has_next) {
+      issue_w(k + 1, (k + 1) % Sh::NWB);
+      issue_halo(k + 1);
+      __builtin_amdgcn_sched_barrier(0);
+    }
+    compute(k);
+    if (has_next) {
+      if constexpr (Sh::NHB == 1) drain_and_barrier();
+      write_halo((k + 1) % Sh::NHB);
+      drain_and_barrier();
+    }
+  }
+
+  const TileOut t{a.y, wset_ptr(a.bias, a.b_gs, n, a.wdiv), a.res, a.act, a.ps, a.accum, a.Cout, a.Ho, a.Wo, a.gmask, a.gmask_act};
+  store_mfma_tile<MT, 1>(acc, t, n, cbi * MT * 32, oy0, 4, ox0, oy0 + wave, lo, hi);
+}
+
+template <int MT, bool VEC2>
+static int launch_s2split(ConvK2 k, hipStream_t st) {
+  using Sh = S2Shape<MT>;
+  auto kern = conv2d_s2split_kernel<MT, VEC2>;
+  static PerDeviceOnce attr_once;
+  set_dyn_lds_once(attr_once, (const void*)kern, Sh::LDS_BYTES);
+  k.tiles_x = ceil_div(k.Wo, 32); k.tiles_y = ceil_div(k.Ho, 4); k.ntiles = k.tiles_x * k.tiles_y * k.N;
+  k.ncb = ceil_div(k.Cout, 32 * MT);
+  k.tiles_per_xcd = ceil_div(k.ntiles, 8);
+  k.nitems = k.tiles_per_xcd * 8 * k.ncb;
+  hipLaunchKernelGGL(kern, dim3(k.nitems), dim3(256), Sh::LDS_BYTES, st, k);
+  return check_launch("conv2d_s2split_kernel");
+}
+
+int conv2d_s2split_launch(const ConvK2& k, int mt, hipStream_t st) {
+  DVSR_REQUIRE(k.c1 == 0 && k.c0 % 8 == 0 && k.Cout % 32 == 0 && k.pad == 1 && !k.in_ps && !k.in_dil && (mt == 1 || mt == 2) &&
+                   k.Ho == (k.H - 1) / 2 + 1 && k.Wo == (k.W - 1) / 2 + 1,
+               DVSR_ERR_UNSUPPORTED, "conv2d_packed: the stride-2 split kernel needs one plain input in 8-channel chunks, Cout %% 32 == 0 "
+               "and pad 1 (c0=%d c1=%d Cout=%d pad=%d)", k.c0, k.c1, k.Cout, k.pad);
+  const bool vec2 = k.W % 2 == 0 && k.x0_bs % 2 == 0 && ((uintptr_t)k.x0 & 7) == 0;
+  if (mt == 2) return vec2 ? launch_s2split<2, true>(k, st) : launch_s2split<2, false>(k, st);
+  return vec2 ? launch_s2split<1, true>(k, st) : launch_s2split<1, false>(k, st);
+}
+
+}
diff --git a/dynavsr_amd/csrc/conv2d_v2.hip b/dynavsr_amd/csrc/conv2d_v2.hip
--- a/dynavsr_amd/csrc/conv2d_v2.hip
+++ b/dynavsr_amd/csrc/conv2d_v2.hip
@@ -206,7 +206,8 @@
 #pragma unroll
     for (int c = 0; c < CC; ++c) {
 #pragma unroll
-      for (int e = 0; e < E; ++e) rin[c][e] = *reinterpret_cast<const float*>(p + eoffb[e]);
+      for (int e = 0; e < E; ++e)
+        if (!(DVSR_ABLATE(a) & 2)) rin[c][e] = *reinterpret_cast<const float*>(p + eoffb[e]);
       if (c + 1 < CC) {
         const size_t inc = (c & 1) == 0 ? inc0 : ((c & 3) == 1 ? inc1 : inc3);
         p += (cbase + c + 1 < Ctot) ? inc : 0;
@@ -301,6 +302,7 @@
     if (k < 8) DVSR_STAMP(3 + 4 * k);
     f32x4 A[2][Sh::AG ? 1 : MT][PIECES], Bv[Sh::AG ? 1 : 2][NT][PIECES];
     auto load_ops = [&](int step, int rb) {
+      if (DVSR_ABLATE(a) & 32) return;
       const int tap = step / KQ4, q = step - tap * KQ4;
       const int ty = tap / KS, tx = tap - ty * KS;
 #pragma unroll
@@ -376,8 +378,10 @@
 #pragma unroll
           for (int mt = 0; mt < MT; ++mt)
 #pragma unroll
-            for (int nt = 0; nt < NT; ++nt)
-              acc[mt][nt] = __builtin_amdgcn_mfma_f32_32x32x2f32(A[rb][mt][0][j], Bv[rb][nt][0][j], acc[mt][nt], 0, 0, 0);
+            for (int nt = 0; nt < NT; ++nt) {
+              if (DVSR_ABLATE(a) & 16) asm volatile("" ::"v"(A[rb][mt][0][j]), "v"(Bv[rb][nt][0][j]));
+              else acc[mt][nt] = __builtin_amdgcn_mfma_f32_32x32x2f32(A[rb][mt][0][j], Bv[rb][nt][0][j], acc[mt][nt], 0, 0, 0);
+            }
       }
     }
     if (HAS_NEXT) __syncthreads();
@@ -400,6 +404,7 @@
   block(a.nchunks - 1, std::false_type{});
 
   DVSR_STAMP(40);
+  if ((DVSR_ABLATE(a) & 1) && acc[0][0][0] != 12345.f) return;
   const TileOut t{a.y, wset_ptr(a.bias, a.b_gs, n, a.wdiv), a.res, a.act, a.ps, a.accum, a.Cout, a.Ho, a.Wo, a.gmask, a.gmask_act};
   store_mfma_tile<MT, NT>(acc, t, n, cbi * MT * 32, oy0, TH, ox0, oy0 + NT * wave, lo, hi);
 #ifdef DVSR_CONV_TRACE
@@ -873,6 +878,14 @@
   }
   if ((wino_on == 2 || f2.cost < direct) && device_lds_optin() >= (size_t)155 * 1024)
     return ConvGeo{8, f2.th, 2, 0, wino3_on ? ConvKernel::WINO_F2_BF16 : ConvKernel::WINO_F2};
+  return g;
+}
+
+ConvGeo conv2_s2_split(ConvGeo g, int ks, int stride, int pad, int c0, int c1, int Cout, bool plain) {
+  if (!int_or(getenv("DVSR_CONV_S2_SPLIT"), 1)) return g;
+  if (ks == 3 && stride == 2 && pad == 1 && plain && c1 == 0 && c0 > 0 && c0 % 8 == 0 && Cout % 32 == 0 && g.kernel == ConvKernel::REG &&
+      g.bf == 0 && g.cc == 8 && g.th == 4)
+    g.bf = 2;
   return g;
 }
 
@@ -987,6 +1000,11 @@
   ConvK2 k;
   int rc = conv2d_packed_prepare(d, wp, ex, geo, &k);
   if (rc) return rc;
+  if (is_s2_split(geo)) {
+    DVSR_REQUIRE(d.ks == 3 && d.stride == 2 && geo.th == 4, DVSR_ERR_UNSUPPORTED, "conv2d_packed: the stride-2 split kernel runs 3x3 / "
+                 "stride 2 launches on 4-row tiles (ks=%d stride=%d th=%d)", d.ks, d.stride, geo.th);
+    return conv2d_s2split_launch(k, geo.mt, st);
+  }
   if (geo.bf) {
     DVSR_REQUIRE((d.ks == 3 || (d.ks == 2 && geo.bf == 2)) && d.stride == 1 && geo.cc == 16 && (geo.th == 4 || (geo.bf == 2 && geo.th == 8)),
                  DVSR_ERR_UNSUPPORTED,
@@ -1044,6 +1062,13 @@
   return o;
 }
 OpPack op_pack_for(const dvsr_conv2d_desc& d, int Cout, int Ctot) {
+  if (d.ks == 3 && d.stride == 2) {
+    OpPack o;
+    const int Ho = (d.H + 2 * d.pad - 3) / 2 + 1, Wo = (d.W + 2 * d.pad - 3) / 2 + 1;
+    o.geo = dvsr::conv2_s2_split(dvsr::conv2_choose(3, 2, d.N, Ho, Wo, Cout, Ctot, dvsr::ALLOW_NONE), 3, 2, d.pad, d.c0, d.c1, Cout, true);
+    o.floats = dvsr::conv2_pack_floats(3, Cout, Ctot, o.geo);
+    return o;
+  }
   const bool big = d.ks == 7 || d.ks == 9;
   const bool aligned = (((uintptr_t)d.x0 | (uintptr_t)d.x1) & 15) == 0 && (big ? (d.c1 == 0 || d.c0 % 8 == 0) : (d.c0 % 8 == 0 && d.c1 % 8 == 0)) &&
                        d.x0_bstride % 4 == 0 && d.x1_bstride % 4 == 0 && (d.H * d.W) % 4 == 0;
@@ -1051,8 +1076,9 @@
 }
 int op_run(const dvsr_conv2d_desc& d, const dvsr::ConvExtra& ex, int Cout, int Ctot, void* ws, size_t bytes, hipStream_t st) {
   using namespace dvsr;
-  DVSR_REQUIRE((d.ks == 1 || d.ks == 3 || d.ks == 7 || d.ks == 9) && d.stride == 1 && d.pad == d.ks / 2, DVSR_ERR_UNSUPPORTED,
-               "conv2d (packed): ks=%d stride=%d pad=%d (1x1 / 3x3 / 7x7 / 9x9, stride 1, pad ks/2)", d.ks, d.stride, d.pad);
+  DVSR_REQUIRE((d.ks == 1 || d.ks == 3 || d.ks == 7 || d.ks == 9) && (d.stride == 1 || (d.ks == 3 && d.stride == 2 && !d.pre)) && d.pad == d.ks / 2,
+               DVSR_ERR_UNSUPPORTED, "conv2d (packed): ks=%d stride=%d pad=%d (1x1 / 3x3 / 7x7 / 9x9, stride 1 -- 3x3 also stride 2 --, pad ks/2)",
+               d.ks, d.stride, d.pad);
   const OpPack o = op_pack_for(d, Cout, Ctot);
   DVSR_REQUIRE(d.ks <= 3 || o.geo.kernel == ConvKernel::ROW_SPLIT, DVSR_ERR_UNSUPPORTED, "conv2d (packed): this %dx%d convolution is not eligible for the "
                "row-split kernel (dvsr_conv2d_packed_geometry): use dvsr_conv2d_forward / _backward", d.ks, d.ks);
@@ -1074,6 +1100,9 @@
 extern "C" size_t dvsr_conv2d_packed_workspace_bytes(const dvsr_conv2d_desc* d) {
   if (!d || (d->ks != 1 && d->ks != 3 && d->ks != 7 && d->ks != 9)) return 0;
   const int ctot = d->c0 + d->c1;
+  if (d->ks == 3 && d->stride == 2)
+    return std::max(dvsr::conv2_pack_floats(3, d->Cout, ctot, 8, 0, dvsr::PackLayout::INTERLEAVED),
+                    dvsr::conv2_pack_floats(3, d->Cout, ctot, 8, 0, dvsr::PackLayout::DCN_SPLIT)) * sizeof(float);
   const size_t a = op_pack(d->ks, 1, d->ks / 2, d->N, d->H, d->W, d->Cout, ctot, true).floats;
   const size_t b = op_pack(d->ks, 1, d->ks / 2, d->N, d->H, d->W, ctot, d->Cout, true).floats;
   const size_t c = op_pack(d->ks, 1, d->ks / 2, d->N, d->H, d->W, d->Cout, ctot, false).floats;
@@ -1085,11 +1114,19 @@
 }
 
 extern "C" int dvsr_conv2d_packed_geometry(const dvsr_conv2d_desc* d, int geo[4]) {
-  DVSR_REQUIRE(d && geo && (d->ks == 1 || d->ks == 3 || d->ks == 7 || d->ks == 9) && d->stride == 1 && d->pad == d->ks / 2,
-               DVSR_ERR_INVALID, "conv2d_packed_geometry: 1x1 / 3x3 / 7x7 / 9x9 stride-1 descriptors only");
+  DVSR_REQUIRE(d && geo && (d->ks == 1 || d->ks == 3 || d->ks == 7 || d->ks == 9) && (d->stride == 1 || (d->ks == 3 && d->stride == 2)) &&
+                   d->pad == d->ks / 2,
+               DVSR_ERR_INVALID, "conv2d_packed_geometry: 1x1 / 3x3 / 7x7 / 9x9 stride-1 and 3x3 stride-2 descriptors only");
   const OpPack o = op_pack_for(*d, d->Cout, d->c0 + d->c1);
   geo[0] = o.geo.cc; geo[1] = o.geo.th; geo[2] = o.geo.mt; geo[3] = static_cast<int>(o.geo.kernel);
   return DVSR_OK;
+}
+
+extern "C" int dvsr_conv2d_packed_pipe(const dvsr_conv2d_desc* d) {
+  if (!d || !((d->ks == 1 || d->ks == 3 || d->ks == 7 || d->ks == 9) && (d->stride == 1 || (d->ks == 3 && d->stride == 2)) && d->pad == d->ks / 2))
+    return -1;
+  const OpPack o = op_pack_for(*d, d->Cout, d->c0 + d->c1);
+  return dvsr::on_bf16_split(o.geo.kernel) ? 2 : o.geo.bf;
 }
 
 extern "C" int dvsr_conv2d_forward_packed(const dvsr_conv2d_desc* d, void* workspace, size_t workspace_bytes,
diff --git a/dynavsr_amd/csrc/engine.hip b/dynavsr_amd/csrc/engine.hip
--- a/dynavsr_amd/csrc/engine.hip
+++ b/dynavsr_amd/csrc/engine.hip
@@ -177,6 +177,10 @@
   if ((fwd_ok & ALLOW_WINO) && !nograd.l[0].pack.geo.bf) {
     const ConvGeo g5 = conv2_choose(ks, o.stride, N, Ho, Wo, Cout, c0 + c1, fwd_ok | ALLOW_WINO_F4 | ALLOW_SHARED_DEVICE);
     if (g5.kernel == ConvKernel::WINO_F4) nograd.l[0] = whole(g5);
+  }
+  if (o.stride == 2 && !p.use_v1 && p.wsets == 1) {
+    const ConvGeo gs = conv2_s2_split(nograd.l[0].pack.geo, ks, o.stride, conv_pad(o), c0, c1, Cout, plain);
+    if (is_s2_split(gs)) nograd.l[0] = whole(gs);
   }
   const Op::LaunchList pair = plan_hoist(o, p, fwd_ok, nograd.l[0]);
   if (pair.n) {
@@ -1195,6 +1199,12 @@
   return o.type == OP_CONV ? o.launches[nograd ? FWD_NOGRAD : FWD_GRAD].n : 1;
 }
 
+extern "C" int dvsr_edvr_op_matrix_pipe(const dvsr_edvr_plan* p, int index, int nograd) {
+  if (!p || index < 0 || index >= (int)p->ops.size() || p->ops[index].type != OP_CONV) return -1;
+  const ConvGeo& g = p->ops[index].launches[nograd ? FWD_NOGRAD : FWD_GRAD].primary().pack.geo;
+  return on_bf16_split(g.kernel) ? 2 : g.bf;
+}
+
 static int plan_work(const dvsr_edvr_plan* p, double* out9, FwdMode mode) {
   DVSR_REQUIRE(p && out9, DVSR_ERR_INVALID, "edvr_plan_work: null argument");
   double fa = 0, fe = 0, ba = 0, be = 0, fby = 0, f32p[2] = {0, 0}, bfp[2] = {0, 0};
diff --git a/dynavsr_amd/csrc/kernels.h b/dynavsr_amd/csrc/kernels.h
--- a/dynavsr_amd/csrc/kernels.h
+++ b/dynavsr_amd/csrc/kernels.h
@@ -75,19 +75,25 @@
 size_t conv2_pack_floats(int ks, int Cout, int Ctot, int cc, int bf, PackLayout layout);
 PackEntry conv2_pack_entry(const float* w, float* P, int ks, int Cout, int Ctot, int cc, int bf, PackLayout layout, int wt = 0,
                            int w_ctot = 0, int w_coff = 0);
+constexpr bool is_s2_split(const ConvGeo& g) { return g.kernel == ConvKernel::REG && g.bf == 2 && g.cc == 8; }
 inline size_t conv2_pack_floats(int ks, int Cout, int Ctot, const ConvGeo& g) {
+  if (is_s2_split(g)) return conv2_pack_floats(ks, Cout, Ctot, 8, 0, PackLayout::DCN_SPLIT);
   return conv2_pack_floats(ks, Cout, Ctot, g.cc, g.bf, pack_layout(g.kernel));
 }
 inline PackEntry conv2_pack_entry(const float* w, float* P, int ks, int Cout, int Ctot, const ConvGeo& g, int wt = 0, int w_ctot = 0,
                                   int w_coff = 0) {
+  if (is_s2_split(g)) return conv2_pack_entry(w, P, ks, Cout, Ctot, 8, 0, PackLayout::DCN_SPLIT, wt, w_ctot, w_coff);
   return conv2_pack_entry(w, P, ks, Cout, Ctot, g.cc, g.bf, pack_layout(g.kernel), wt, w_ctot, w_coff);
 }
+ConvGeo conv2_s2_split(ConvGeo g, int ks, int stride, int pad, int c0, int c1, int Cout, bool plain);
 double conv2_f4_occupied_cycles(int N, int Ho, int Wo, int Cout, int Ctot, int th);
 int pack_weights_wino_run(const PackTable& t, hipStream_t st);
 int pack_weights_wino3_run(const PackTable& t, hipStream_t st);
 int pack_weights_wino5_run(const PackTable& t, hipStream_t st);
 int conv2d_packed_run(const dvsr_conv2d_desc& d, const float* wp, const ConvExtra& ex, const ConvGeo& geo,
                       hipStream_t st);
+struct ConvK2;
+int conv2d_s2split_launch(const ConvK2& k, int mt, hipStream_t st);
 
 bool conv1x1_dual_ok(const float* x, const float* w0, const float* w1, const float* y0, const float* y1, int Cin, long long HW);
 int conv1x1_dual_run(const float* x, const float* w0, const float* b0, const float* w1, const float* b1, float* y0, float* y1,
diff --git a/dynavsr_amd/engine.py b/dynavsr_amd/engine.py
--- a/dynavsr_amd/engine.py
+++ b/dynavsr_amd/engine.py
@@ -7,7 +7,7 @@
 
 _plans = {}
 _GEOMETRY_ENV = ("DVSR_CONV_WINO", "DVSR_CONV_WINO3", "DVSR_CONV_WINO5", "DVSR_CONV_V1", "DVSR_EST_SPLIT", "DVSR_EST_SPLIT2", "DVSR_FUSE_ACT_BWD",
-                 "DVSR_BWD_STREAMS", "DVSR_PCD_HOIST")
+                 "DVSR_BWD_STREAMS", "DVSR_PCD_HOIST", "DVSR_CONV_S2_SPLIT")
 _PROCESS_ENV = ("DVSR_CONV_LDS", "DVSR_CONV_LAST_MFMA", "DVSR_SPLIT_TH8_FROM", "DVSR_WGRAD_SPLIT3",
                 "DVSR_WGRAD_WIDE", "DVSR_WGRAD_S3V", "DVSR_WGRAD_S3_KYS_BELOW", "DVSR_WGRAD_S3_WGS", "DVSR_WGRAD_S3W", "DVSR_DCN_FWD", "DVSR_DCN_BWD",
                 "DVSR_EST_FUSE_PAD", "DVSR_FUSE_RES_BWD", "DVSR_BWD_FORK_EVERY", "DVSR_BWD_PROBE", "DVSR_TSA_DUAL", "DVSR_TSA_V",
diff --git a/include/dynavsr_hip.h b/include/dynavsr_hip.h
--- a/include/dynavsr_hip.h
+++ b/include/dynavsr_hip.h
@@ -120,6 +120,7 @@
 int dvsr_edvr_plan_work(const dvsr_edvr_plan* plan, double* out9);
 int dvsr_edvr_plan_work_nograd(const dvsr_edvr_plan* plan, double* out9);
 int dvsr_edvr_op_launch_count(const dvsr_edvr_plan* plan, int index, int nograd);
+int dvsr_edvr_op_matrix_pipe(const dvsr_edvr_plan* plan, int index, int nograd);
 int dvsr_side_stream_overlaps(dvsr_stream_t stream);
 int dvsr_edvr_op_output(const dvsr_edvr_plan* plan, int index, int which, int* in_arena, long long* offset_floats,
                         long long* numel);
@@ -291,6 +292,7 @@
 int dvsr_conv2d_dgrad_packed(const dvsr_conv2d_desc* d, const float* gy, float* gx0, void* workspace,
                              size_t workspace_bytes, dvsr_stream_t stream);
 int dvsr_conv2d_packed_geometry(const dvsr_conv2d_desc* d, int geo[4]);
+int dvsr_conv2d_packed_pipe(const dvsr_conv2d_desc* d);
 
 int dvsr_conv2d_wgrad_bf16(const dvsr_conv2d_desc* d, const float* gy, float* gw, float* gb, void* workspace,
                            size_t workspace_bytes, dvsr_stream_t stream);
```

Result: no change. 261.1 frames/s (median of 6 runs) (+0.7%).
